# SuperScientificSoftwareLaboratory/DASP

Measured on AMD Instinct MI355X. Metric: SpMV GFLOP/s (f64), higher is better.
Workload: dtype f64; 1 GPU; HV15R synthetic stand-in (seeded; SuiteSparse dims/row statistics), A=1, x=1; rows=2017169, cols=2017169, nnz=275454726, partition=single GPU, generator_rev=26e32ff958e7, y_candidates=1

## Files before the change

dasp_amd/_lib.py:

```python
import ctypes as C
import os
import subprocess

_HERE = os.path.dirname(os.path.abspath(__file__))
SO_PATH = os.environ.get("DASP_AMD_SO") or os.path.join(_HERE, "libdasp_amd.so")


class DaspError(RuntimeError):
    def __init__(self, status, msg):
        super().__init__("dasp status %d: %s" % (status, msg))
        self.status = status


class Options(C.Structure):
    _fields_ = [
        ("threshold", C.c_double), ("block_longest", C.c_int), ("y_order", C.c_int), ("long_piece", C.c_int),
        ("host_threads", C.c_int), ("n_parts", C.c_int), ("part_bounds", C.POINTER(C.c_int)), ("part_stride", C.c_int),
        ("x_window", C.c_int), ("row_window", C.c_int), ("cid16", C.c_int), ("stream_policy", C.c_int),
        ("col_panels", C.c_int), ("slab_max_len", C.c_int), ("x_window_hybrid", C.c_int), ("piece_min_len", C.c_int),
        ("chunk_pairs", C.c_int), ("cid8", C.c_int), ("short_seg", C.c_int), ("row_tile_max", C.c_int), ("sort_columns", C.c_int),
        ("two_phase", C.c_int), ("tp_col_block", C.c_int), ("tp_row_block", C.c_int), ("long_cb", C.c_int),
        ("value_map", C.c_int),
    ]

    def _tp_exact_cell(self):
        return C.c_int.from_address(C.addressof(self) + Options.value_map.offset + C.sizeof(C.c_int))

    @property
    def tp_exact(self):
        return self._tp_exact_cell().value

    @tp_exact.setter
    def tp_exact(self, v):
        self._tp_exact_cell().value = int(v)


assert Options.value_map.offset + 2 * C.sizeof(C.c_int) <= C.sizeof(Options), "dasp_options_t::tp_exact must lie inside the Python mirror of the struct"


class Stats(C.Structure):
    _fields_ = [(n, C.c_int) for n in (
        "precision rowA colA nnzA short_row_1 common_13 short_row_3 short_row_4 short_row_2 row_long row_block "
        "row_zero nnz_short nnz_long origin_nnz_reg nnz_irreg rowloop").split()] + [
        ("fill0_nnz_short", C.c_longlong), ("fill0_nnz_long", C.c_longlong), ("fill0_nnz_reg", C.c_longlong),
        ("rate_fill0", C.c_double), ("data_X", C.c_longlong), ("data_origin1", C.c_longlong),
        ("n_med_blocks", C.c_int), ("n_long_pieces", C.c_int), ("n_long_multi", C.c_int), ("n_short_tiles", C.c_int),
        ("n_workgroups", C.c_int), ("pre_ms", C.c_double),
        ("x_window_on", C.c_int), ("n_windows", C.c_int), ("n_windows_lds", C.c_int), ("lds_bytes", C.c_int),
        ("row_window", C.c_int), ("window_nnz_frac", C.c_double), ("cid16_on", C.c_int),
        ("n_col_panels", C.c_int), ("x_window_hybrid", C.c_int), ("med_rows_as_pieces", C.c_int), ("chunk_pairs", C.c_int), ("cid8_chunks", C.c_int), ("short_seg", C.c_int),
        ("row_tile_max", C.c_int), ("n_row_tiles", C.c_int), ("row_tile_nnz", C.c_longlong),
        ("two_phase", C.c_int), ("tp_col_block", C.c_int), ("tp_row_blocks", C.c_int), ("tp_units", C.c_int), ("tp_segments", C.c_longlong), ("tp_seg_elems", C.c_int),
        ("lcb_rows", C.c_int), ("lcb_col_block", C.c_int), ("lcb_units", C.c_int), ("lcb_elems", C.c_longlong),
        ("ref_fill0_nnz_short", C.c_longlong), ("ref_fill0_nnz_long", C.c_longlong), ("ref_fill0_nnz_reg", C.c_longlong), ("ref_data_X", C.c_longlong),
        ("ref_nnz_irreg", C.c_int), ("ref_origin_nnz_reg", C.c_int), ("ref_blocknum", C.c_int), ("ref_warp_number", C.c_int), ("ref_rate_fill0", C.c_double)]

    def as_dict(self):
        return {n: getattr(self, n) for n, _ in self._fields_}


class MgInfo(C.Structure):
    _fields_ = [(n, C.c_int) for n in "precision n_gpus rank rowA colA row_begin row_end stride".split()] + [
        ("nnz_own", C.c_longlong), ("nnz_other", C.c_longlong), ("overlap", C.c_int), ("has_comm", C.c_int), ("square", C.c_int), ("stream_memops", C.c_int), ("fused_step", C.c_int), ("exchange", C.c_int)]

    def as_dict(self):
        return {n: getattr(self, n) for n, _ in self._fields_}


def build(force=False):
    src = os.path.join(_HERE, "csrc")
    if force:
        subprocess.check_call(["make", "-C", src, "-s", "clean"])
    subprocess.check_call(["make", "-C", src, "-s", "-j8", "all"])
    return SO_PATH


_lib = None


def _preload_hip_runtime():
    import importlib.util
    import sys
    if "torch" in sys.modules:
        return
    try:
        spec = importlib.util.find_spec("torch")
    except (ImportError, ValueError):
        spec = None
    if spec is None or not spec.origin:
        return
# ... 5 lines not shown
            pass


def lib():
    global _lib
    if _lib is not None:
        return _lib
    if not os.path.exists(SO_PATH):
        raise ImportError(
            "dasp_amd: %s is missing. Build it with `python -c 'import __graft_entry__ as g; g.build()'` "
            "(hipcc --offload-arch=gfx950). There is no fallback implementation." % SO_PATH)
    _preload_hip_runtime()
    L = C.CDLL(SO_PATH)
    ip, vp = C.POINTER(C.c_int), C.c_void_p
    L.dasp_last_error.restype = C.c_char_p
    L.dasp_version.restype = C.c_char_p
    L.dasp_free.argtypes = [vp]
    L.dasp_options_default.argtypes = [C.POINTER(Options)]
    L.dasp_mmio_allinone_f64.argtypes = [ip, ip, ip, ip, C.POINTER(ip), C.POINTER(ip), C.POINTER(C.POINTER(C.c_double)), C.c_char_p]
    L.dasp_mmio_allinone_f16.argtypes = [ip, ip, ip, ip, C.POINTER(ip), C.POINTER(ip), C.POINTER(C.POINTER(C.c_uint16)), C.c_char_p]
    L.dasp_csr_save.argtypes = [C.c_char_p, C.c_int, C.c_int, C.c_int, C.c_int, C.c_int, vp, vp, vp]
    L.dasp_csr_load.argtypes = [C.c_char_p, C.c_int, ip, ip, ip, ip, C.POINTER(ip), C.POINTER(ip), C.POINTER(vp)]
    L.dasp_plan_create.argtypes = [C.POINTER(vp), C.c_int, C.c_int, C.c_int, C.c_int, vp, vp, vp, C.POINTER(Options)]
    L.dasp_plan_create_device.argtypes = [C.POINTER(vp), C.c_int, C.c_int, C.c_int, C.c_int, vp, vp, vp, C.POINTER(Options)]
    L.dasp_plan_download_array.argtypes = [vp, C.c_char_p, vp, C.c_size_t]
    L.dasp_plan_destroy.argtypes = [vp]
    L.dasp_plan_save.argtypes = [vp, C.c_char_p]
    L.dasp_plan_load.argtypes = [C.POINTER(vp), C.c_char_p]
    L.dasp_plan_order.argtypes = [vp]
    L.dasp_plan_order.restype = ip
    L.dasp_plan_stats.argtypes = [vp, C.POINTER(Stats)]
    L.dasp_plan_y_order.argtypes = [vp]
    L.dasp_plan_x_len.argtypes = [vp]
    L.dasp_plan_x_len.restype = C.c_longlong
    L.dasp_plan_host_array.argtypes = [vp, C.c_char_p, C.POINTER(vp), ip]
    L.dasp_plan_host_array.restype = C.c_longlong
    L.dasp_plan_panel_count.argtypes = [vp]
    L.dasp_plan_panel.argtypes = [vp, C.c_int]
    L.dasp_plan_panel.restype = vp
    L.dasp_plan_panel_range.argtypes = [vp, C.c_int, ip, ip]
    L.dasp_plan_upload.argtypes = [vp]
    L.dasp_plan_drop_host.argtypes = [vp]
    L.dasp_plan_update_values.argtypes = [vp, vp, vp]
    L.dasp_plan_update_values_host.argtypes = [vp, vp]
    L.dasp_plan_value_map_slots.argtypes = [vp]
    L.dasp_plan_value_map_slots.restype = C.c_longlong
    if hasattr(L, "dasp_plan_csr_fetch_bytes"):
        L.dasp_plan_csr_fetch_bytes.argtypes = [vp]
        L.dasp_plan_csr_fetch_bytes.restype = C.c_longlong
    if hasattr(L, "dasp_plan_shared_ids"):
        L.dasp_plan_shared_ids.argtypes = [vp, C.POINTER(C.c_longlong), C.POINTER(C.c_longlong), ip]
        L.dasp_plan_shared_ids_export.argtypes = [vp, C.c_char_p, vp, C.c_size_t]
        L.dasp_plan_shared_ids_export.restype = C.c_longlong
    L.dasp_plan_set_stream_policy.argtypes = [vp, C.c_int]
    if hasattr(L, "dasp_plan_set_tp_exact"):
        L.dasp_plan_set_tp_exact.argtypes = [vp, C.c_int]
        L.dasp_plan_tp_exact.argtypes = [vp]
        L.dasp_tp_exact_dot_f16.argtypes = [vp, vp, C.c_longlong, C.c_int, C.c_uint16, C.POINTER(C.c_uint16)]
    if hasattr(L, "dasp_plan_set_hub_exact"):
        L.dasp_plan_set_hub_exact.argtypes = [vp, C.c_int]
        L.dasp_plan_hub_exact.argtypes = [vp]
    if hasattr(L, "dasp_plan_set_f32_vectors"):
        fp = C.POINTER(C.c_float)
        L.dasp_plan_set_f32_vectors.argtypes = [vp, C.c_int]
        L.dasp_plan_f32_vectors.argtypes = [vp]
        L.dasp_plan_spmv_f32.argtypes = [vp, fp, fp, vp]
        L.dasp_plan_spmv_acc_f32.argtypes = [vp, fp, fp, vp]
    if hasattr(L, "dasp_debug_plan_kernel"):
        L.dasp_debug_spmv_variant.argtypes = [C.c_int, C.c_uint]
        L.dasp_debug_spmv_variant.restype = C.c_char_p
        L.dasp_debug_plan_kernel.argtypes = [vp]
        L.dasp_debug_plan_kernel.restype = C.c_char_p
    L.dasp_plan_spmv.argtypes = [vp, vp, vp, vp]
    L.dasp_plan_spmv_acc.argtypes = [vp, vp, vp, vp]
    L.dasp_plan_time.argtypes = [vp, vp, vp, vp, C.c_int, C.c_int, C.POINTER(C.c_double), C.POINTER(C.c_double)]
    L.dasp_plan_time_each.argtypes = [vp, vp, vp, vp, C.c_int, C.c_int, vp]
    L.dasp_plan_time_graph.argtypes = [vp, vp, vp, vp, C.c_int, C.c_int, C.c_int, C.POINTER(C.c_double), C.POINTER(C.c_double)]
    L.dasp_spmv_all_f64.argtypes = [C.c_char_p, vp, vp, vp, vp, vp, vp, C.c_int, C.c_int, C.c_int, C.c_int, C.c_double, C.c_int]
    L.dasp_spmv_all_f16.argtypes = L.dasp_spmv_all_f64.argtypes
    L.dasp_partition_rows.argtypes = [C.c_int, vp, C.c_int, vp]
    L.dasp_selftest_mfma.argtypes = []
    L.dasp_plan_tune_placement.argtypes = [vp, C.c_int, vp, vp, C.POINTER(C.c_double), C.POINTER(C.c_double)]
    L.dasp_mg_unique_id.argtypes = [vp]
    L.dasp_mg_plan_create.argtypes = [C.POINTER(vp), C.c_int, C.c_int, C.c_int, C.c_int, C.c_int, vp, vp, vp, vp, C.POINTER(Options), C.c_int]
    L.dasp_mg_destroy.argtypes = [vp]
    L.dasp_mg_upload.argtypes = [vp]
    L.dasp_mg_comm_init.argtypes = [vp, vp]
    L.dasp_mg_set_x.argtypes = [vp, vp]
    L.dasp_mg_spmv.argtypes = [vp, vp]
    L.dasp_mg_product.argtypes = [vp, vp]
    L.dasp_mg_allgather.argtypes = [vp, vp]
    L.dasp_mg_wait.argtypes = [vp, vp]
    L.dasp_mg_get_y.argtypes = [vp, vp]
    L.dasp_mg_get_y_local.argtypes = [vp, vp]
    for f in (L.dasp_mg_y_local, L.dasp_mg_gathered, L.dasp_mg_x):
        f.argtypes = [vp]
        f.restype = vp
    L.dasp_mg_subplan.argtypes = [vp, C.c_int]
    L.dasp_mg_subplan.restype = vp
    L.dasp_mg_info.argtypes = [vp, C.POINTER(MgInfo)]
    L.dasp_mg_check.argtypes = [vp]
    L.dasp_mg_set_fused.argtypes = [vp, C.c_int]
    L.dasp_mg_set_fake_exchange.argtypes = [vp, C.c_int, C.c_int, vp]
    L.dasp_mg_push_export.argtypes = [vp, vp]
    L.dasp_mg_push_connect.argtypes = [vp, vp]
    L.dasp_mg_set_exchange.argtypes = [vp, C.c_int]
    L.dasp_mg_push_loopback.argtypes = [vp]
    L.dasp_mg_reserved_stream.argtypes = [vp, C.c_int]
    L.dasp_mg_reserved_stream.restype = vp
    L.dasp_synth_dims.argtypes = [C.c_char_p, C.c_double, ip, ip]
    L.dasp_synth_generator.argtypes = [C.c_char_p]
    L.dasp_synth_generator.restype = C.c_char_p
    L.dasp_synth_row_lengths.argtypes = [C.c_char_p, C.c_double, C.c_int, C.c_int, vp]
    L.dasp_synth_rows.argtypes = [C.c_char_p, C.c_double, C.c_int, C.c_int, vp, vp]
    _lib = L
    return L


def check(rc):
    if rc != 0:
        raise DaspError(rc, lib().dasp_last_error().decode("utf-8", "replace"))


EXPORTS = (
    "dasp_last_error dasp_version dasp_mmio_allinone_f64 dasp_mmio_allinone_f16 dasp_free dasp_csr_save dasp_csr_load dasp_options_default "
    "dasp_plan_create dasp_plan_create_device dasp_plan_download_array dasp_plan_destroy dasp_plan_save dasp_plan_load dasp_plan_order dasp_plan_stats dasp_plan_y_order dasp_plan_x_len dasp_plan_panel_count dasp_plan_panel dasp_plan_panel_range dasp_plan_host_array dasp_plan_upload dasp_plan_tune_placement "
    "dasp_plan_drop_host dasp_plan_update_values dasp_plan_update_values_host dasp_plan_value_map_slots dasp_plan_csr_fetch_bytes dasp_plan_shared_ids dasp_plan_shared_ids_export dasp_plan_set_stream_policy dasp_plan_set_tp_exact dasp_plan_tp_exact dasp_plan_set_hub_exact dasp_plan_hub_exact dasp_tp_exact_dot_f16 dasp_plan_spmv dasp_plan_spmv_acc dasp_plan_set_f32_vectors dasp_plan_f32_vectors dasp_plan_spmv_f32 dasp_plan_spmv_acc_f32 dasp_plan_time dasp_plan_time_each dasp_plan_time_graph dasp_spmv_all_f64 dasp_spmv_all_f16 dasp_partition_rows "
    "dasp_selftest_mfma dasp_synth_dims dasp_synth_generator dasp_synth_row_lengths dasp_synth_rows "
    "dasp_mg_unique_id dasp_mg_plan_create dasp_mg_destroy dasp_mg_upload dasp_mg_comm_init dasp_mg_set_x dasp_mg_spmv dasp_mg_product dasp_mg_allgather "
    "dasp_mg_wait dasp_mg_get_y dasp_mg_get_y_local dasp_mg_y_local dasp_mg_gathered dasp_mg_x dasp_mg_subplan dasp_mg_info dasp_mg_check dasp_mg_set_fused dasp_mg_set_fake_exchange "
    "dasp_mg_push_export dasp_mg_push_connect dasp_mg_set_exchange dasp_mg_push_loopback dasp_mg_reserved_stream").split()
```

dasp_amd/api.py:

```python
import ctypes as C
import os

import numpy as np

from . import _lib
from ._lib import DaspError, Options, Stats

Y_PERMUTED, Y_NATURAL = 0, 1


def _vp(a):
    return a.ctypes.data_as(C.c_void_p)


def _dtype(precision):
    if precision == 64:
        return np.float64
    if precision == 16:
        return np.float16
    raise ValueError("precision must be 64 or 16")


def mmio_allinone(filename, precision=64):
    L = _lib.lib()
    ip = C.POINTER(C.c_int)
    m, n, nnz, sym = C.c_int(), C.c_int(), C.c_int(), C.c_int()
    rp, ci = ip(), ip()
    if precision == 64:
        v = C.POINTER(C.c_double)()
        rc = L.dasp_mmio_allinone_f64(C.byref(m), C.byref(n), C.byref(nnz), C.byref(sym), C.byref(rp), C.byref(ci), C.byref(v), os.fsencode(filename))
    else:
        v = C.POINTER(C.c_uint16)()
        rc = L.dasp_mmio_allinone_f16(C.byref(m), C.byref(n), C.byref(nnz), C.byref(sym), C.byref(rp), C.byref(ci), C.byref(v), os.fsencode(filename))
    _lib.check(rc)
    k = nnz.value
    row_ptr = np.ctypeslib.as_array(rp, (m.value + 1,)).copy()
    col_idx = np.ctypeslib.as_array(ci, (max(k, 1),))[:k].copy()
    raw = np.ctypeslib.as_array(v, (max(k, 1),))[:k].copy()
    val = raw if precision == 64 else raw.view(np.float16)
    for q in (rp, ci, v):
        L.dasp_free(C.cast(q, C.c_void_p))
    return m.value, n.value, k, sym.value, row_ptr, col_idx, val


def csr_save(path, row_ptr, col_idx, val, n_cols, is_symmetric=0, precision=64):
    rp = np.ascontiguousarray(row_ptr, np.int32)
    ci = np.ascontiguousarray(col_idx, np.int32)
    v = np.ascontiguousarray(val, _dtype(precision))
    _lib.check(_lib.lib().dasp_csr_save(os.fsencode(path), precision, rp.size - 1, int(n_cols), int(ci.size), int(is_symmetric), _vp(rp), _vp(ci), _vp(v)))


def csr_load(path, precision=64):
    L = _lib.lib()
    ip = C.POINTER(C.c_int)
    m, n, nnz, sym = C.c_int(), C.c_int(), C.c_int(), C.c_int()
    rp, ci, v = ip(), ip(), C.c_void_p()
    _lib.check(L.dasp_csr_load(os.fsencode(path), precision, C.byref(m), C.byref(n), C.byref(nnz), C.byref(sym), C.byref(rp), C.byref(ci), C.byref(v)))
    k = nnz.value
    row_ptr = np.ctypeslib.as_array(rp, (m.value + 1,)).copy()
    col_idx = np.ctypeslib.as_array(ci, (max(k, 1),))[:k].copy()
    ct = C.c_double if precision == 64 else C.c_uint16
    raw = np.ctypeslib.as_array(C.cast(v, C.POINTER(ct)), (max(k, 1),))[:k].copy()
    val = raw if precision == 64 else raw.view(np.float16)
    for q in (C.cast(rp, C.c_void_p), C.cast(ci, C.c_void_p), v):
        L.dasp_free(q)
    return m.value, n.value, k, sym.value, row_ptr, col_idx, val


class Plan:

    def __init__(self, csrRowPtr, csrColIdx, csrVal, colA, precision=64, threshold=0.75, block_longest=256,
                 y_order=Y_PERMUTED, long_piece=0, host_threads=0, part_bounds=None, part_stride=0, x_window=0, row_window=0, cid16=0, stream_policy=0,
                 col_panels=0, slab_max_len=0, x_window_hybrid=0, piece_min_len=0, chunk_pairs=0, cid8=0, short_seg=0, row_tile_max=0, sort_columns=0,
                 two_phase=0, tp_col_block=0, tp_row_block=0, long_cb=0, value_map=0, tp_exact=0):
        L = _lib.lib()
        self.precision = precision
        dt = _dtype(precision)
        rp = np.ascontiguousarray(csrRowPtr, np.int32)
        ci = np.ascontiguousarray(csrColIdx, np.int32)
        v = np.ascontiguousarray(csrVal, dt)
        self.rowA, self.colA, self.nnzA = rp.size - 1, int(colA), int(ci.size)
        opt = Options()
        L.dasp_options_default(C.byref(opt))
        opt.threshold, opt.block_longest, opt.y_order = threshold, block_longest, y_order
        opt.long_piece, opt.host_threads = long_piece, host_threads
        opt.x_window, opt.row_window, opt.cid16, opt.stream_policy = x_window, row_window, cid16, stream_policy
        opt.col_panels, opt.slab_max_len, opt.x_window_hybrid, opt.piece_min_len = col_panels, slab_max_len, x_window_hybrid, piece_min_len
        opt.chunk_pairs, opt.cid8, opt.short_seg, opt.row_tile_max, opt.sort_columns = chunk_pairs, cid8, short_seg, row_tile_max, sort_columns
        opt.two_phase, opt.tp_col_block, opt.tp_row_block, opt.long_cb = two_phase, tp_col_block, tp_row_block, long_cb
        opt.value_map, opt.tp_exact = value_map, tp_exact
        self._pb = None
        if part_bounds is not None:
            self._pb = np.ascontiguousarray(part_bounds, np.int32)
            opt.n_parts = self._pb.size - 1
            opt.part_bounds = self._pb.ctypes.data_as(C.POINTER(C.c_int))
            opt.part_stride = int(part_stride)
        self._h = C.c_void_p()
        _lib.check(L.dasp_plan_create(C.byref(self._h), precision, self.rowA, self.colA, self.nnzA, _vp(rp), _vp(ci), _vp(v), C.byref(opt)))
        self.y_order = y_order
        self.x_len = self.colA if part_bounds is None else (self._pb.size - 1) * int(part_stride)

    @classmethod
    def from_device(cls, d_row_ptr, d_col_idx, d_val, rowA, colA, nnzA, precision=64, threshold=0.75, block_longest=256,
                    y_order=Y_PERMUTED, long_piece=0, part_bounds=None, part_stride=0, x_window=0, row_window=0, cid16=0, col_panels=0, slab_max_len=0,
                    x_window_hybrid=0, piece_min_len=0, chunk_pairs=0, cid8=0, short_seg=0, row_tile_max=0, sort_columns=0, two_phase=0, tp_col_block=0, tp_row_block=0, long_cb=0,
                    value_map=0, tp_exact=0):
        L = _lib.lib()
        self = cls.__new__(cls)
        self.precision, self.rowA, self.colA, self.nnzA = precision, int(rowA), int(colA), int(nnzA)
        opt = Options()
        L.dasp_options_default(C.byref(opt))
        opt.threshold, opt.block_longest, opt.y_order, opt.long_piece = threshold, block_longest, y_order, long_piece
        opt.x_window, opt.row_window, opt.cid16, opt.col_panels = x_window, row_window, cid16, col_panels
        opt.slab_max_len, opt.x_window_hybrid, opt.piece_min_len = slab_max_len, x_window_hybrid, piece_min_len
        opt.chunk_pairs, opt.cid8, opt.short_seg, opt.row_tile_max, opt.sort_columns = chunk_pairs, cid8, short_seg, row_tile_max, sort_columns
        opt.two_phase, opt.tp_col_block, opt.tp_row_block, opt.long_cb = two_phase, tp_col_block, tp_row_block, long_cb
        opt.value_map, opt.tp_exact = value_map, tp_exact
        self._pb = None
        if part_bounds is not None:
            self._pb = np.ascontiguousarray(part_bounds, np.int32)
            opt.n_parts, opt.part_stride = self._pb.size - 1, int(part_stride)
            opt.part_bounds = self._pb.ctypes.data_as(C.POINTER(C.c_int))
        self._h = C.c_void_p()
        _lib.check(L.dasp_plan_create_device(C.byref(self._h), precision, self.rowA, self.colA, self.nnzA, C.c_void_p(d_row_ptr),
                                             C.c_void_p(d_col_idx), C.c_void_p(d_val), C.byref(opt)))
        self.y_order = y_order
        self.x_len = int(L.dasp_plan_x_len(self._h))
        return self

    def device_array(self, name, count, dtype):
        out = np.empty(count, dtype)
        _lib.check(_lib.lib().dasp_plan_download_array(self._h, name.encode(), _vp(out), out.nbytes))
        return out

    def save(self, path):
        _lib.check(_lib.lib().dasp_plan_save(self._h, os.fsencode(path)))

    @classmethod
    def load(cls, path):
        self = cls.__new__(cls)
        self._h = C.c_void_p()
        self._pb = None
        _lib.check(_lib.lib().dasp_plan_load(C.byref(self._h), os.fsencode(path)))
        st = self.stats
        self.precision, self.rowA, self.colA, self.nnzA = st["precision"], st["rowA"], st["colA"], st["nnzA"]
        self.y_order = _lib.lib().dasp_plan_y_order(self._h)
        self.x_len = int(_lib.lib().dasp_plan_x_len(self._h))
        return self

    @property
    def order_rid(self):
        if self.rowA == 0:
            return np.zeros(0, np.int32)
        p = _lib.lib().dasp_plan_order(self._h)
        return np.ctypeslib.as_array(p, (max(self.rowA, 1),))[: self.rowA].copy()

    @property
    def stats(self):
        s = Stats()
        _lib.check(_lib.lib().dasp_plan_stats(self._h, C.byref(s)))
        return s.as_dict()

    @property
    def n_panels(self):
        return int(_lib.lib().dasp_plan_panel_count(self._h))

    def panel(self, k):
        L = _lib.lib()
        h = L.dasp_plan_panel(self._h, k)
        if not h:
# ... 14 lines not shown
            _lib.check(int(n))
        if name in ("med_cid16", "long_cid16", "rt_start", "tp_lrow", "tp_lcol", "lcb_lcol"):
            dt = np.uint16
        elif name.endswith("_val_map"):
            dt = np.uint32
        elif name == "rt_mask":
            dt = np.uint64
        elif name == "med_cid8":
            dt = np.uint8
        elif eb.value == 4:
            dt = np.int32
        else:
            dt = np.float64 if eb.value == 8 else np.float16
        if n == 0:
            return np.zeros(0, dt)
        buf = (C.c_char * (n * eb.value)).from_address(ptr.value)
        return np.frombuffer(buf, dtype=dt).copy()

    def upload(self):
        _lib.check(_lib.lib().dasp_plan_upload(self._h))
        return self

    def tune_placement(self, trials=0, dX=0, dY=0):
        a, b = C.c_double(), C.c_double()
        _lib.check(_lib.lib().dasp_plan_tune_placement(self._h, int(trials), C.c_void_p(dX or None), C.c_void_p(dY or None), C.byref(a), C.byref(b)))
        return a.value, b.value

    def drop_host(self):
        _lib.check(_lib.lib().dasp_plan_drop_host(self._h))

    def update_values(self, csrVal):
        v = np.ascontiguousarray(csrVal, _dtype(self.precision))
        if v.size != self.nnzA:
            raise ValueError("update_values: %d values for a plan of %d nonzeros" % (v.size, self.nnzA))
        _lib.check(_lib.lib().dasp_plan_update_values_host(self._h, _vp(v)))

    def update_values_device(self, d_val, stream=0):
        _lib.check(_lib.lib().dasp_plan_update_values(self._h, C.c_void_p(d_val), C.c_void_p(stream)))

    @property
    def csr_fetch_bytes(self):
        n = int(_lib.lib().dasp_plan_csr_fetch_bytes(self._h))
        if n < 0:
            _lib.check(n)
        return n

    def shared_ids(self):
        pb, sb, use = C.c_longlong(0), C.c_longlong(0), C.c_int(0)
        rc = _lib.lib().dasp_plan_shared_ids(self._h, C.byref(pb), C.byref(sb), C.byref(use))
        if rc < 0:
            _lib.check(rc)
        return {"available": bool(rc), "paired_id_bytes": int(pb.value), "shared_bytes": int(sb.value), "in_use": bool(use.value)}

    def shared_ids_export(self):
        out = []
        for what in (b"plane", b"table"):
            n = int(_lib.lib().dasp_plan_shared_ids_export(self._h, what, None, 0))
            if n < 0:
                _lib.check(n)
            a = np.empty(n // 4, np.uint32)
            n2 = int(_lib.lib().dasp_plan_shared_ids_export(self._h, what, a.ctypes.data_as(C.c_void_p), a.nbytes))
            if n2 < 0:
                _lib.check(n2)
            out.append(a)
        return out[0], out[1].reshape(-1, 4)

    @property
    def value_map_slots(self):
        n = int(_lib.lib().dasp_plan_value_map_slots(self._h))
        if n < 0:
            _lib.check(n)
        return n

    def kernel_variant(self):
        name = _lib.lib().dasp_debug_plan_kernel(self._h)
        if name is None:
            raise _lib.DaspError(-22, _lib.lib().dasp_last_error().decode("utf-8", "replace"))
        return name.decode()

    def set_stream_policy(self, policy):
        _lib.check(_lib.lib().dasp_plan_set_stream_policy(self._h, int(policy)))

    def set_tp_exact(self, on):
        _lib.check(_lib.lib().dasp_plan_set_tp_exact(self._h, int(on)))

    @property
    def tp_exact(self):
        return int(_lib.lib().dasp_plan_tp_exact(self._h))

    def set_hub_exact(self, on):
        _lib.check(_lib.lib().dasp_plan_set_hub_exact(self._h, int(on)))

    @property
    def hub_exact(self):
        return int(_lib.lib().dasp_plan_hub_exact(self._h))

    def spmv(self, dX, dY, stream=0, accumulate=False):
        f = _lib.lib().dasp_plan_spmv_acc if accumulate else _lib.lib().dasp_plan_spmv
        _lib.check(f(self._h, C.c_void_p(dX), C.c_void_p(dY), C.c_void_p(stream)))

    def set_f32_vectors(self, on):
        _lib.check(_lib.lib().dasp_plan_set_f32_vectors(self._h, int(on)))

    @property
    def f32_vectors(self):
        return int(_lib.lib().dasp_plan_f32_vectors(self._h))
# ... 110 lines not shown
```

dasp_amd/csrc/capi.cpp:

```cpp
#include <hip/hip_runtime_api.h>

#include <algorithm>
#include <cstdio>
#include <cstdlib>
#include <cstring>
#include <exception>
#include <memory>
#include <new>
#include <string>
#include <sys/stat.h>
#include <vector>

#include "plan.hpp"
#include "device.hpp"
#include "tp_exact.hpp"

namespace dasp {
const char *last_error_cstr();
int upload_plan(Plan &p);
int tune_placement(Plan &p, int trials, const void *dX, void *dY, double *ms_first, double *ms_kept);
int launch_spmv(Plan &p, const void *dX, void *dY, void *stream, bool accumulate);
int time_spmv_each(Plan &p, const void *dX, void *dY, void *stream, int warmup, int iters, float *ms_each);
int time_spmv(Plan &p, const void *dX, void *dY, void *stream, int warmup, int iters, double *wall_ms, double *event_ms);
int time_spmv_graph(Plan &p, const void *dX, void *dY, void *stream, int warmup, int iters, int batch, double *wall_ms, double *event_ms);
// ... 25 lines not shown
    std::memset(o, 0, sizeof *o);
    o->threshold = 0.75;
    o->block_longest = 256;
    o->y_order = DASP_Y_PERMUTED;
}

int dasp_mmio_allinone_f64(int *m, int *n, int *nnz, int *isSymmetric, int **csrRowPtr, int **csrColIdx,
                           double **csrVal, const char *filename)
{
    void *v = nullptr;
    int rc = guarded("dasp_mmio_allinone_f64", [&] { return load_mtx(filename, 64, m, n, nnz, isSymmetric, csrRowPtr, csrColIdx, &v); });
    if (rc == DASP_OK) *csrVal = static_cast<double *>(v);
    return rc;
}

int dasp_mmio_allinone_f16(int *m, int *n, int *nnz, int *isSymmetric, int **csrRowPtr, int **csrColIdx,
                           uint16_t **csrVal, const char *filename)
{
    void *v = nullptr;
    int rc = guarded("dasp_mmio_allinone_f16", [&] { return load_mtx(filename, 16, m, n, nnz, isSymmetric, csrRowPtr, csrColIdx, &v); });
    if (rc == DASP_OK) *csrVal = static_cast<uint16_t *>(v);
    return rc;
}

int dasp_csr_save(const char *path, int precision, int m, int n, int nnz, int isSymmetric, const int *csrRowPtr,
                  const int *csrColIdx, const void *csrVal)
{
    return guarded("dasp_csr_save", [&] { return save_csr_bin(path, precision, m, n, nnz, isSymmetric, csrRowPtr, csrColIdx, csrVal); });
}

int dasp_csr_load(const char *path, int precision, int *m, int *n, int *nnz, int *isSymmetric, int **csrRowPtr,
                  int **csrColIdx, void **csrVal)
{
    return guarded("dasp_csr_load", [&] { return load_csr_bin(path, precision, m, n, nnz, isSymmetric, csrRowPtr, csrColIdx, csrVal); });
}

static int normalise_options(Plan &p, const dasp_options_t *opt, int colA)
{
    if (opt) p.opt = *opt; else dasp_options_default(&p.opt);
    if (!(p.opt.threshold > 0)) p.opt.threshold = 0.75;
    if (p.opt.block_longest < 6) p.opt.block_longest = 256;
    if (p.opt.n_parts > 0) {
        if (!p.opt.part_bounds || p.opt.part_stride <= 0) { set_error("bad column partition"); return DASP_ERR_ARG; }
        p.part_bounds.assign(p.opt.part_bounds, p.opt.part_bounds + p.opt.n_parts + 1);
        if (p.part_bounds.front() != 0 || p.part_bounds.back() != colA) { set_error("part_bounds must span [0,colA]"); return DASP_ERR_ARG; }
        for (int g = 0; g < p.opt.n_parts; ++g)
            if (p.part_bounds[g + 1] < p.part_bounds[g] || p.part_bounds[g + 1] - p.part_bounds[g] > p.opt.part_stride) {
                set_error("part_bounds not monotone or wider than part_stride"); return DASP_ERR_ARG;
            }
        p.opt.part_bounds = p.part_bounds.data();
    } else { p.opt.n_parts = 0; p.opt.part_bounds = nullptr; }
    if (p.opt.value_map != 0 && p.opt.value_map != 1) { set_error("value_map must be 0 or 1"); return DASP_ERR_ARG; }
    if (p.opt.tp_exact != 0 && p.opt.tp_exact != 1) { set_error("tp_exact must be 0 or 1"); return DASP_ERR_ARG; }
    return DASP_OK;
}

int dasp_plan_create(dasp_plan_t **out, int precision, int rowA, int colA, int nnzA, const int *rp, const int *ci,
                     const void *val, const dasp_options_t *opt)
{
    if (!out) return DASP_ERR_ARG;
    *out = nullptr;
    if ((precision != 64 && precision != 16) || rowA < 0 || colA < 0 || nnzA < 0 || !rp || (nnzA > 0 && (!ci || !val))) {
        set_error("dasp_plan_create: bad arguments");
        return DASP_ERR_ARG;
    }
    return guarded("dasp_plan_create", [&] {
        std::unique_ptr<dasp_plan> h(new dasp_plan());
        Plan &p = h->impl;
        p.precision = precision; p.m = rowA; p.n = colA; p.nnz = nnzA;
        if (int rc = normalise_options(p, opt, colA)) return rc;
        if (int rc = build_plan(p, rp, ci, val)) return rc;
        if (int rc = set_tp_exact(p, p.opt.tp_exact)) return rc;
        *out = h.release();
        return (int)DASP_OK;
    });
}

int dasp_plan_create_device(dasp_plan_t **out, int precision, int rowA, int colA, int nnzA, const int *dRowPtr, const int *dColIdx,
                            const void *dVal, const dasp_options_t *opt)
{
    if (!out) return DASP_ERR_ARG;
    *out = nullptr;
    if ((precision != 64 && precision != 16) || rowA < 0 || colA < 0 || nnzA < 0 || !dRowPtr || (nnzA > 0 && (!dColIdx || !dVal))) {
        set_error("dasp_plan_create_device: bad arguments");
        return DASP_ERR_ARG;
    }
    return guarded("dasp_plan_create_device", [&] {
        std::vector<int> rp((size_t)rowA + 1);
        if (hipMemcpy(rp.data(), dRowPtr, sizeof(int) * ((size_t)rowA + 1), hipMemcpyDeviceToHost) != hipSuccess) {
            set_error("cannot read the device row pointer (no HIP device, or not a device pointer)");
            return (int)DASP_ERR_HIP;
        }
        std::unique_ptr<dasp_plan> h(new dasp_plan());
        Plan &p = h->impl;
        p.precision = precision; p.m = rowA; p.n = colA; p.nnz = nnzA;
        if (int rc = normalise_options(p, opt, colA)) return rc;
        const DevCsr dev{dRowPtr, dColIdx, dVal};
        if (int rc = build_plan(p, rp.data(), nullptr, nullptr, &dev)) return rc;
        if (int rc = set_tp_exact(p, p.opt.tp_exact)) return rc;
        *out = h.release();
        return (int)DASP_OK;
    });
}

int dasp_plan_download_array(dasp_plan_t *plan, const char *name, void *dst, size_t bytes)
{
// ... 121 lines not shown
    if (n == "rt_ptr") return ints(p.rt_ptr);
    if (n == "rt_start") { *ptr = p.rt_start.data(); *elem_bytes = 2; return (long long)p.rt_start.size(); }
    if (n == "rt_mask") { *ptr = p.rt_mask.data(); *elem_bytes = 8; return (long long)p.rt_mask.size(); }
    if (n == "lcb_row_dst") return ints(p.lcb.row_dst);
    if (n == "lcb_row_id") return ints(p.lcb.row_id);
    if (n == "lcb_ptr") return ints(p.lcb.ptr);
    if (n == "lcb_unit") return ints(p.lcb.unit);
    if (n == "lcb_val") return vals(p.lcb.val);
    if (n == "lcb_lcol") { *ptr = p.lcb.lcol.data(); *elem_bytes = 2; return (long long)p.lcb.lcol.size(); }
    if (n == "tp_rb_row0") return ints(p.tp.rb_row0);
    if (n == "tp_rb_seg0") return ints(p.tp.rb_seg0);
    if (n == "tp_unit") return ints(p.tp.unit);
    if (n == "tp_dst") return ints(p.tp.dst);
    if (n == "tp_val") return vals(p.tp.val);
    if (n == "tp_lrow") { *ptr = p.tp.lrow.data(); *elem_bytes = 2; return (long long)p.tp.lrow.size(); }
    if (n == "tp_lcol") { *ptr = p.tp.lcol.data(); *elem_bytes = 2; return (long long)p.tp.lcol.size(); }
    if (n == "short_groups") {
        static thread_local std::vector<int> flat;
        flat.clear();
        for (int g = 0; g < kNumShortGroups; ++g) {
            const ShortGroup &G = p.grp[g];
            const int row[15] = {G.len, G.count, G.tiles, G.tile0, (int)(G.elem_off & 0xffffffffll), (int)(G.elem_off >> 32),
                                 G.map.split, G.map.base[0], G.map.base[1], G.map.grp[0], G.map.grp[1], G.map.off[0], G.map.off[1], G.seg, G.rpt};
            flat.insert(flat.end(), row, row + 15);
        }
        return ints(flat);
    }
    set_error("unknown host array: " + n);
    return DASP_ERR_ARG;
}

long long dasp_plan_csr_fetch_bytes(const dasp_plan_t *plan) { return plan ? plan->impl.csr_fetch_bytes : (long long)DASP_ERR_ARG; }

int dasp_plan_shared_ids(const dasp_plan_t *plan, long long *paired_id_bytes, long long *shared_bytes, int *in_use)
{
    if (!plan) return DASP_ERR_ARG;
    const Plan &p = plan->impl;
    if (paired_id_bytes) *paired_id_bytes = 0;
    if (shared_bytes) *shared_bytes = 0;
    if (in_use) *in_use = p.dev && p.sh_in_use ? 1 : 0;
    return guarded("dasp_plan_shared_ids", [&] {
        long long pb = 0, sb = 0;
        if (!p.sh_known) {
            SharedIds sh;
            (void)derive_shared_ids(p, sh);
            p.sh_paired_bytes = sh.paired_id_bytes; p.sh_shared_bytes = sh.shared_bytes; p.sh_known = true;
        }
        pb = p.sh_paired_bytes; sb = p.sh_shared_bytes;
        if (pb == 0) return 0;
        if (paired_id_bytes) *paired_id_bytes = pb;
        if (shared_bytes) *shared_bytes = sb;
        return 1;
    });
}

long long dasp_plan_shared_ids_export(const dasp_plan_t *plan, const char *what, void *dst, size_t bytes)
{
    if (!plan || !what) return DASP_ERR_ARG;
    long long need = 0;
    const int rc = guarded("dasp_plan_shared_ids_export", [&] {
        const bool plane = std::strcmp(what, "plane") == 0;
        if (!plane && std::strcmp(what, "table") != 0) { set_error("dasp_plan_shared_ids_export: \"plane\" or \"table\""); return (int)DASP_ERR_ARG; }
        SharedIds sh;
        if (!derive_shared_ids(plan->impl, sh)) { set_error("the plan has no shared id plane (f64 with 16-bit ids, host arrays present, at least one pipelined block)"); return (int)DASP_ERR_STATE; }
        const std::vector<uint32_t> &v = plane ? sh.plane : sh.table;
        need = (long long)v.size() * 4;
        if (dst && bytes >= (size_t)need && need > 0) std::memcpy(dst, v.data(), (size_t)need);
        return (int)DASP_OK;
    });
    return rc != DASP_OK ? (long long)rc : need;
}

int dasp_plan_upload(dasp_plan_t *plan)
{
    if (!plan) return DASP_ERR_ARG;
    return guarded("dasp_plan_upload", [&] { return upload_plan(plan->impl); });
}

int dasp_plan_tune_placement(dasp_plan_t *plan, int trials, const void *dX, void *dY, double *ms_first, double *ms_kept)
{
    if (!plan) return DASP_ERR_ARG;
    if (!plan->impl.dev) { set_error("plan not uploaded"); return DASP_ERR_STATE; }
    return guarded("dasp_plan_tune_placement", [&] { return tune_placement(plan->impl, trials, dX, dY, ms_first, ms_kept); });
}

int dasp_plan_drop_host(dasp_plan_t *plan)
{
    if (!plan) return DASP_ERR_ARG;
    Plan &p = plan->impl;
    if (!p.dev) { set_error("upload the plan before dropping its host arrays"); return DASP_ERR_STATE; }
    auto dropc = [](raw_vector<char> &v) { raw_vector<char>().swap(v); };
    auto dropi = [](raw_vector<int> &v) { raw_vector<int>().swap(v); };
    dropc(p.long_val); dropi(p.long_cid); raw_vector<uint16_t>().swap(p.long_cid16); dropc(p.med_val); dropi(p.med_cid); raw_vector<uint16_t>().swap(p.med_cid16); raw_vector<uint8_t>().swap(p.med_cid8);
    dropc(p.irr_val); dropi(p.irr_cid); dropc(p.short_val); dropi(p.short_cid); dropc(p.rt_val); dropi(p.rt_cid);
    dropc(p.lcb.val); raw_vector<uint16_t>().swap(p.lcb.lcol);
    dropc(p.tp.val); raw_vector<uint16_t>().swap(p.tp.lrow); raw_vector<uint16_t>().swap(p.tp.lcol); std::vector<int>().swap(p.tp.dst);
    for (auto *m : {&p.long_map, &p.med_map, &p.irr_map, &p.short_map, &p.rt_map, &p.tp.map, &p.lcb.map}) std::vector<uint32_t>().swap(*m);
    p.host_dropped = true;
    for (auto &h : p.panels) if (int rc = dasp_plan_drop_host(h.get())) return rc;
    return DASP_OK;
}

int dasp_plan_set_stream_policy(dasp_plan_t *plan, int policy)
{
    if (!plan) return DASP_ERR_ARG;
    return set_stream_policy(plan->impl, policy);
// ... 212 lines not shown
```

dasp_amd/csrc/devpack.hip:

```cpp
#include <hip/hip_runtime.h>
#include <hipcub/hipcub.hpp>

#include <memory>
#include <thread>

#include <algorithm>
#include <chrono>
#include <cstdio>
#include <cstdlib>
#include <cstring>
#include <string>
#include <type_traits>
#include <vector>

#include "device.hpp"

namespace dasp {

#define HIP_TRYP(expr)                                                                         \
    do {                                                                                       \
        hipError_t e_ = (expr);                                                                \
        if (e_ != hipSuccess) {                                                                \
            set_error(std::string(#expr) + ": " + hipGetErrorString(e_));                      \
            return e_ == hipErrorNoDevice ? DASP_ERR_NO_DEVICE : DASP_ERR_HIP;                 \
// ... 89 lines not shown
__global__ void k_iota1(unsigned *out, long long n)
{
    for (long long i = (long long)blockIdx.x * blockDim.x + threadIdx.x; i < n; i += (long long)gridDim.x * blockDim.x) out[i] = (unsigned)(i + 1);
}

template <class T>
__global__ void k_pack_long(const int *rp, const int *ci, const T *val, const int *ridL, const long long *startL, int nlong, RemapDev remap,
                            T *lv, int *lc, const unsigned *src, unsigned *lm )
{
    const int lane = threadIdx.x & 63, i = blockIdx.x * (blockDim.x >> 6) + (threadIdx.x >> 6);
    if (i >= nlong) return;
    const int r = ridL[i], a0 = rp[r], len = rp[r + 1] - a0;
    const long long at = startL[i], padded = startL[i + 1] - at;
    for (long long j = lane; j < padded; j += 64) {
        const bool in = j < len;
        lv[at + j] = in ? val[a0 + j] : (T)0;
        lc[at + j] = in ? remap(ci[a0 + j]) : -1;
        if (lm) lm[at + j] = in ? map_of(src, a0 + j) : 0u;
    }
}

__global__ void k_long_cid16(const int *lc, const int *piece_ptr, int *piece_c16, int np, int CH, int *lbase, unsigned short *lc16)
{
    const int lane = threadIdx.x & 63, q = blockIdx.x * (blockDim.x >> 6) + (threadIdx.x >> 6);
    if (q >= np) return;
    const int e0 = piece_ptr[q], e1 = piece_ptr[q + 1], c0 = piece_c16[2 * q];
    bool narrow = true;
    for (int e = e0, c = c0; e < e1; e += CH, ++c) {
        int lo = 2147483647, hi = -1;
        for (int j = e + lane; j < min(e + CH, e1); j += 64) { const int col = lc[j]; if (col >= 0) { lo = min(lo, col); hi = max(hi, col); } }
        for (int d = 32; d > 0; d >>= 1) { lo = min(lo, __shfl_xor(lo, d)); hi = max(hi, __shfl_xor(hi, d)); }
        const int b = hi < 0 ? 0 : lo;
        if (lane == 0) lbase[c] = b;
        if (hi >= 0 && (long long)hi - lo > 65534) narrow = false;
        for (int j = e + lane; j < min(e + CH, e1); j += 64) { const int col = lc[j]; lc16[j] = col < 0 ? kLongPad16 : (unsigned short)(col - b); }
    }
    narrow = narrow && e1 - e0 >= kLong16MinChunks * CH;
    if (lane == 0) piece_c16[2 * q + 1] = narrow ? 1 : 0;
    if (!narrow) for (int j = e0 + lane; j < e1; j += 64) lc16[j] = 0;
}

template <class T, bool C16>
__global__ void k_pack_medium(const int *rp, const int *ci, const T *val, const int *ridM, const int *lenM, const int *med_ptr,
                              const int *irr_ptr, int nmed, int nb, RemapDev remap, T *mv, int *mc, unsigned short *mc16, int *mbase,
                              T *iv, int *ic, int pair_mode, const int *c8ptr, unsigned char *mc8, int *korig,
                              const int *win_cmin, const int *win_len, int bpw ,
                              const unsigned *src, unsigned *mm, unsigned *im )
{
    constexpr int K = sizeof(T) == 8 ? 4 : 16, CH = kMedRows * K, VPL = CH / 64;
    const int lane = threadIdx.x & 63, b = blockIdx.x * (blockDim.x >> 6) + (threadIdx.x >> 6);
    if (b >= nb) return;
    const int c0 = med_ptr[b], nc = med_ptr[b + 1] - c0;
    const int r0 = b * kMedRows;
    const int nt_b = (irr_ptr[r0 + 1] - irr_ptr[r0] + K - 1) / K;
    const int npair = med_npair(nc, nt_b, (int)sizeof(T), pair_mode);
    const bool oneshot = med_oneshot64(nc, nt_b);
    const int rr = lane & 15, kq = lane >> 4, r = r0 + rr;
    const bool row_ok = r < nmed;
    const int a0 = row_ok ? rp[ridM[r]] : 0, len = row_ok ? lenM[r] : 0;
    int n8 = 0, a8 = 0, a16 = 0; size_t e8 = 0, e16 = (size_t)c0 * CH;
    if constexpr (C16) { n8 = c8ptr[b + 1] - c8ptr[b]; e8 = (size_t)c8ptr[b] * CH; e16 = ((size_t)c0 - (size_t)c8ptr[b]) * CH; }
    for (int c = 0; c < nc; ++c) {
        int col[VPL]; T v[VPL]; unsigned ms[VPL];
        int lo = 2147483647, hi = -1;
#pragma unroll
        for (int q = 0; q < VPL; ++q) {
            const int i = c * K + (VPL == 1 ? kq : 4 * kq + q);
            const bool in = row_ok && i < len;
            v[q] = in ? val[a0 + i] : (T)0;
            col[q] = in ? remap(ci[a0 + i]) : -1;
            ms[q] = in && mm ? map_of(src, a0 + i) : 0u;
            if (in) { lo = min(lo, col[q]); hi = max(hi, col[q]); }
        }
        if constexpr (C16) {
            lo = wave_min(lo); hi = wave_max(hi);
            const bool narrow = c < npair && c < 64 && a8 < n8 && hi >= 0 && hi - lo <= 254;
            if (lo == 2147483647) lo = 0;
            if (bpw > 0 && win_len[b / bpw] > 0) lo = win_cmin[b / bpw];
            const int pos = c >= npair ? c : narrow ? a8++ : n8 + a16++;
            if (lane == 0) { mbase[c0 + pos] = lo; korig[c0 + pos] = c; }
            const size_t at = (size_t)c0 * CH + med_elem_index(npair, pos, lane, 0, VPL, CH);
#pragma unroll
            for (int q = 0; q < VPL; ++q) {
                mv[at + q] = v[q];
                if (mm) mm[at + q] = ms[q];
                if (pos < n8) mc8[e8 + med_cid8_index(pos, lane, CH, oneshot)] = col[q] < 0 ? (unsigned char)0xFF : (unsigned char)(col[q] - lo);
                else mc16[e16 + med_elem_index(npair - n8, pos - n8, lane, q, VPL, CH)] = col[q] < 0 ? (unsigned short)0xFFFF : (unsigned short)(col[q] - lo);
            }
        } else {
            const size_t at = (size_t)c0 * CH + med_elem_index(npair, c, lane, 0, VPL, CH);
#pragma unroll
            for (int q = 0; q < VPL; ++q) { mv[at + q] = v[q]; mc[at + q] = col[q]; if (mm) mm[at + q] = ms[q]; }
        }
    }
    if (row_ok) {
        const int t0 = irr_ptr[r], tl = irr_ptr[r + 1] - t0;
        for (int j = kq; j < tl; j += 4) {
            iv[t0 + j] = val[a0 + len - tl + j]; ic[t0 + j] = remap(ci[a0 + len - tl + j]);
            if (im) im[t0 + j] = map_of(src, a0 + len - tl + j);
        }
    }
}

template <class T>
__global__ void k_pack_short(const int *rp, const int *ci, const T *val, const int *list, int count, int tiles, int L, long long elem_off,
                             int SR, int seg, RemapDev remap, T *sv, int *sc, const unsigned *src, unsigned *sm )
{
    const long long n = (long long)tiles * short_tile_elems(seg != 0, L, SR);
    for (long long e = (long long)blockIdx.x * blockDim.x + threadIdx.x; e < n; e += (long long)gridDim.x * blockDim.x) {
        long long t; int k; bool in;
        if (seg) {
// ... 1262 lines not shown
```

dasp_amd/csrc/multigpu.cpp:

```cpp
#include <hip/hip_runtime_api.h>
#include <hip/hip_ext.h>
#include <rccl/rccl.h>

#include <dlfcn.h>

#include <algorithm>
#include <chrono>
#include <cstdlib>
#include <cstring>
#include <exception>
#include <memory>
#include <mutex>
#include <new>
#include <string>
#include <thread>
#include <vector>

#include <unistd.h>

#include "plan.hpp"
#include "device.hpp"
#include "mgx.hpp"

using namespace dasp;
// ... 215 lines not shown
        if (xg && xg != yg) (void)hipFree(xg);
        if (own) dasp_plan_destroy(own);
        if (other) dasp_plan_destroy(other);
    }
};

namespace {

template <class T>
void split_by_owner(int m, const int *rp, const int *ci, const T *val, int lo, int hi, int threads,
                    std::vector<int> &rpO, std::vector<int> &ciO, std::vector<T> &vO,
                    std::vector<int> &rpR, std::vector<int> &ciR, std::vector<T> &vR)
{
    rpO.assign((size_t)m + 1, 0); rpR.assign((size_t)m + 1, 0);
    auto par = [&](auto f) {
        const int parts = std::max(1, std::min(threads, m / 4096 + 1));
        std::vector<std::thread> th;
        for (int t = 0; t < parts; ++t) {
            const int b = (int)((long long)m * t / parts), e = (int)((long long)m * (t + 1) / parts);
            th.emplace_back([=] { f(b, e); });
        }
        for (auto &x : th) x.join();
    };
    par([&](int b, int e) {
        for (int i = b; i < e; ++i) {
            int o = 0;
            for (int j = rp[i]; j < rp[i + 1]; ++j) o += ci[j] >= lo && ci[j] < hi;
            rpO[(size_t)i + 1] = o; rpR[(size_t)i + 1] = rp[i + 1] - rp[i] - o;
        }
    });
    for (int i = 0; i < m; ++i) { rpO[(size_t)i + 1] += rpO[i]; rpR[(size_t)i + 1] += rpR[i]; }
    ciO.resize((size_t)rpO[m]); vO.resize((size_t)rpO[m]); ciR.resize((size_t)rpR[m]); vR.resize((size_t)rpR[m]);
    par([&](int b, int e) {
        for (int i = b; i < e; ++i) {
            int o = rpO[i], r = rpR[i];
            for (int j = rp[i]; j < rp[i + 1]; ++j) {
                if (ci[j] >= lo && ci[j] < hi) { ciO[(size_t)o] = ci[j] - lo; vO[(size_t)o++] = val[j]; }
                else { ciR[(size_t)r] = ci[j]; vR[(size_t)r++] = val[j]; }
            }
        }
    });
}

template <class T>
int create_impl(dasp_mg_plan &g, const int *rp, const int *ci, const T *val, const dasp_options_t *user)
{
    const int m = g.rows();
    const int lo = g.bounds[(size_t)g.rank], hi = g.bounds[(size_t)g.rank + 1];
    dasp_options_t opt;
    if (user) opt = *user; else dasp_options_default(&opt);
    opt.y_order = DASP_Y_NATURAL;
    opt.short_seg = -1;
    opt.two_phase = -1;
    opt.n_parts = 0; opt.part_bounds = nullptr; opt.part_stride = 0;
    opt.tp_exact = 0;
    opt.value_map = 0;
    const int nnz = rp[m];
    if (!g.square) {
        g.nnz_own = nnz; g.nnz_other = 0;
        return dasp_plan_create(&g.own, g.precision, m, g.colA, nnz, rp, ci, val, &opt);
    }
    dasp_options_t part = opt;
    part.n_parts = g.world; part.part_bounds = g.bounds.data(); part.part_stride = g.stride;
    if (!g.overlap) {
        g.nnz_own = nnz; g.nnz_other = 0;
        return dasp_plan_create(&g.own, g.precision, m, g.colA, nnz, rp, ci, val, &part);
    }
    if (g.step2) {
        std::vector<unsigned char> has((size_t)std::max(m, 1), 0);
        long long other = 0;
        for (int i = 0; i < m; ++i) {
            int o = 0;
            for (int j = rp[i]; j < rp[i + 1]; ++j) o += !(ci[j] >= lo && ci[j] < hi);
            has[(size_t)i] = o > 0; other += o;
        }
        g.nnz_own = nnz - other; g.nnz_other = other;
        if (int rc = dasp_plan_create(&g.own, g.precision, m, g.colA, nnz, rp, ci, val, &part)) return rc;
        const Plan &P = g.own->impl;
        if (g.precision == 64 && P.panels.empty() && !P.windowed && P.opt.y_order == DASP_Y_NATURAL) {
            double hot_at = 1.0;
            if (const char *e = std::getenv("DASP_MG_HOT_AT")) hot_at = std::max(0.0, std::min(1.0, std::atof(e)));
            mg_step_marks(P, has.data(), g.mark, g.blk_order, hot_at);
            const int n_pieces = (int)P.piece_dst.size(), wg_long = (n_pieces + kWavesPerWG - 1) / kWavesPerWG;
            const int wg_med = (P.stats.n_med_blocks + kWavesPerWG - 1) / kWavesPerWG;
            int first_hot_med = wg_long + wg_med;
            for (int w = wg_long; w < wg_long + wg_med; ++w) if (g.mark[(size_t)w]) { first_hot_med = w; break; }
            g.wg_list.clear(); g.wg_list.reserve(g.mark.size());
            for (int w = 0; w < first_hot_med; ++w) if (!g.mark[(size_t)w]) g.wg_list.push_back(w);
            g.n_free2 = (int)g.wg_list.size();
            for (size_t w = 0; w < g.mark.size(); ++w) if (g.mark[w]) g.wg_list.push_back((int)w);
            g.n_marked2 = (int)g.wg_list.size() - g.n_free2;
            for (int w = first_hot_med; w < (int)g.mark.size(); ++w) if (!g.mark[(size_t)w]) g.wg_list.push_back(w);
        }
        return DASP_OK;
    }
    std::vector<int> rpO, ciO, rpR, ciR;
    std::vector<T> vO, vR;
    split_by_owner<T>(m, rp, ci, val, lo, hi, resolve_threads(opt.host_threads), rpO, ciO, vO, rpR, ciR, vR);
    g.nnz_own = rpO[(size_t)m]; g.nnz_other = rpR[(size_t)m];
    static const int zero = 0;
    if (int rc = dasp_plan_create(&g.own, g.precision, m, g.stride, rpO[(size_t)m], rpO.data(), ciO.empty() ? &zero : ciO.data(),
                                  vO.empty() ? static_cast<const void *>(&zero) : vO.data(), &opt)) return rc;
    if (part.cid16 == 0 && g.precision == 64 && g.own->impl.cid16) part.cid16 = 1;
    if (g.nnz_other > 0)
        if (int rc = dasp_plan_create(&g.other, g.precision, m, g.colA, rpR[(size_t)m], rpR.data(), ciR.data(), vR.data(), &part)) return rc;
    if (g.other && g.precision == 64 && g.own->impl.panels.empty() && !g.own->impl.windowed && g.own->impl.opt.y_order == DASP_Y_NATURAL) {
// ... 773 lines not shown
```

dasp_amd/csrc/plan.cpp:

```cpp
#include "plan.hpp"

#include <algorithm>
#include <array>
#include <atomic>
#include <chrono>
#include <cstdio>
#include <cstdlib>
#include <cstring>
#include <condition_variable>
#include <functional>
#include <mutex>
#include <thread>

namespace dasp {

static thread_local std::string g_err;
void set_error(const std::string &s) { g_err = s; }
const char *last_error_cstr() { return g_err.c_str(); }

int resolve_threads(int requested)
{
    if (requested > 0) return requested;
    unsigned hc = std::thread::hardware_concurrency();
    if (hc == 0) hc = 1;
// ... 326 lines not shown
    g.fill0_reg = reg; g.nnz_irreg = (int)irr;
    const long long stored = g.fill0_short + g.fill0_long + g.nnz_irreg + g.fill0_reg;
    g.rate_fill0 = nnz > 0 ? (double)(stored - nnz) / nnz : 0.0;
    const long long sv = f16 ? 2 : 8;
    g.data_X = (long long)(m + n) * sv + g.fill0_long * (sv + 4) + (long long)g.warp_number * sv + (long long)(lenL.size() + 1) * 4 + g.fill0_short * (sv + 4) +
               g.fill0_reg * (sv + 4) + (long long)(g.blocknum + 1) * 4 + (long long)(f16 ? (g.nnz_irreg + 1) / 2 * 2 : g.nnz_irreg) * (sv + 4) +
               (long long)(row_block + 1) * 4;
    return g;
}

namespace {
struct LapTimer {
    using clk = std::chrono::steady_clock;
    const char *fmt;
    const clk::time_point t_begin = clk::now();
    const bool verbose = std::getenv("DASP_VERBOSE") != nullptr;
    clk::time_point tick = t_begin;
    explicit LapTimer(const char *f) : fmt(f) {}
    void operator()(const char *what) { if (verbose) { auto now = clk::now(); std::fprintf(stderr, fmt, what, std::chrono::duration<double>(now - tick).count()); tick = now; } }
    double ms() const { return std::chrono::duration<double, std::milli>(clk::now() - t_begin).count(); }
};

template <class T> struct Build {
    Plan &p;
    const int *rp, *ci;
    const T *val;
    const DevCsr *dev;
    const Geometry geo;
    const int m, nnz, threads;
    const bool f16;
    const bool meta_only;
    const bool pack;
    const bool natural, mapped;
    Remap remap;
    LapTimer lap{"[dasp plan] %-28s %.3f s\n"};

    std::vector<int> rid1, rid2, rid3, rid4, rid0;
    int n1 = 0, n3 = 0;
    int n2 = 0, n4 = 0, nz0 = 0, n1_all = 0, n3_all = 0, c13 = 0;
    int row_long = 0;
    int row_block = 0;
    int nnz_short = 0;
    long long nnz_long = 0;
    std::vector<int> ridL;
    raw_vector<int> ridM_in;
    raw_vector<int> ridM, lenM;
    RefGeometry refg;
    int mfma_rows = 0;
    std::vector<std::vector<int>> slab_rows;
    const std::vector<int> *glist[kNumShortGroups] = {};
    double window_frac = 0.0;
    int nsp = 0;
    int rows_as_pieces = 0;
    std::vector<long long> startL;
    int nb = 0;
    long long n_reg = 0;
    int nnz_irreg = 0;

    Build(Plan &p_, const int *rp_, const int *ci_, const T *val_, const DevCsr *dev_, bool meta_only_)
        : p(p_), rp(rp_), ci(ci_), val(val_), dev(dev_), geo(p_.geo), m(p_.m), nnz(p_.nnz), threads(resolve_threads(p_.opt.host_threads)), f16(p_.precision == 16),
          meta_only(meta_only_), pack(!dev_ && !meta_only_), natural(p_.opt.y_order == DASP_Y_NATURAL), mapped(natural && !p_.dst_map.empty())
    {
        remap.n_parts = p.opt.n_parts; remap.stride = p.opt.part_stride; remap.b = p.part_bounds.data();
    }
    Build(const Build &) = delete;
    Build &operator=(const Build &) = delete;
    CsrProbe probe() const { return CsrProbe{p, rp, ci, dev, remap, threads}; }
    int rowdst(int row) const { return mapped ? p.dst_map[row] : row; }
    int ydst(int slot) const { return natural ? rowdst(p.order[slot]) : slot; }
};

bool row_ptr_ends_ok(const int *rp, int m, int nnz)
{
    if (rp[0] != 0 || rp[m] != nnz) { set_error("csrRowPtr[0] != 0 or csrRowPtr[rowA] != nnzA"); return false; }
    return true;
}
}

template <class T> static int validate_csr(Build<T> &bld)
{
    Plan &p = bld.p;
    const int *rp = bld.rp, *ci = bld.ci;
    const DevCsr *dev = bld.dev;
    const int m = bld.m, nnz = bld.nnz, threads = bld.threads;
    if (!row_ptr_ends_ok(rp, m, nnz)) return DASP_ERR_ARG;
    std::atomic<int> bad{0};
    parallel_for(m, threads, 1 << 16, [&](long long b, long long e) {
        for (long long i = b; i < e; ++i) if (rp[i + 1] < rp[i]) { bad = 1; return; }
    });
    const int ncol = p.n;
    if (dev) { if (!bad) { const int rc = devpack_validate(p, *dev); if (rc == DASP_ERR_ARG) bad = 2; else if (rc != DASP_OK) return rc; } }
    else parallel_for(nnz, threads, 1 << 18, [&](long long b, long long e) {
        for (long long i = b; i < e; ++i) if ((unsigned)ci[i] >= (unsigned)ncol) { bad = 2; return; }
    });
    if (bad) { set_error(bad == 1 ? "csrRowPtr not monotone" : "column index out of range"); return DASP_ERR_ARG; }
    bld.lap("validate");
    return DASP_OK;
}

template <class T> struct SortedCsr {
    raw_vector<int> ci;
    raw_vector<T> val;
    raw_vector<uint32_t> src;
    DevCsr dev{nullptr, nullptr, nullptr};
    std::vector<std::shared_ptr<void>> keep;
};
// ... 600 lines not shown
    }

    bld.lap("window decision");
    return DASP_OK;
}

template <class T> static int medium_rows_as_pieces(Build<T> &bld)
{
    Plan &p = bld.p;
    const Geometry &geo = bld.geo;
    const int *rp = bld.rp;
    const int nnz = bld.nnz;
    const bool f16 = bld.f16, meta_only = bld.meta_only;
    std::vector<int> &ridL = bld.ridL;
    raw_vector<int> &ridM = bld.ridM, &lenM = bld.lenM, &ridM_in = bld.ridM_in;
    int &mfma_rows = bld.mfma_rows, &nsp = bld.nsp;
    nsp = 0;
    if (mfma_rows > 0 && !meta_only && p.opt.piece_min_len >= 0 && !p.windowed) {
        int Tmin = p.opt.piece_min_len > 0 ? std::max(5, p.opt.piece_min_len) : 0;
        if (Tmin == 0) {
            const double est_us = (double)nnz * (geo.vbytes + 4) / 5.0e6;
            const int shot = f16 ? 2 : 8, batch = f16 ? 2 : 4;
            auto batches = [&](int L) { const int st = ceil_div(L, geo.med_k); return st <= shot ? 1 : ceil_div(st, batch); };
            const int allowed = std::max(2, (int)(0.25 * est_us / 0.8));
            if (batches(lenM[0]) > allowed) {
                int Lmax = lenM[0];
                while (Lmax > 5 && batches(Lmax) > allowed) --Lmax;
                Tmin = Lmax + 1;
            }
        }
        if (Tmin > 0) {
            const bool forced = p.opt.piece_min_len > 0;
            int cnt = 0; long long k = 0;
            while (cnt < mfma_rows && lenM[cnt] >= Tmin && (forced || (k + lenM[cnt]) * 100 <= 15ll * nnz)) { k += lenM[cnt]; ++cnt; }
            while (cnt > 0 && cnt < mfma_rows && lenM[cnt] == lenM[cnt - 1]) --cnt;
            nsp = cnt;
        }
    }
    if (nsp > 0) {
        const int Tcut = lenM[nsp - 1];
        ridL.insert(ridL.end(), ridM.begin(), ridM.begin() + nsp);
        ridM.erase(ridM.begin(), ridM.begin() + nsp); lenM.erase(lenM.begin(), lenM.begin() + nsp);
        raw_vector<int> keep; keep.reserve(ridM_in.size());
        for (int r : ridM_in) if (rp[r + 1] - rp[r] < Tcut) keep.push_back(r);
        ridM_in.swap(keep);
        mfma_rows -= nsp;
    }
    bld.rows_as_pieces = bld.row_long + nsp;
    p.med_slot0 = bld.rows_as_pieces;
    p.n_mfma_rows = mfma_rows;
    return DASP_OK;
}

template <class T> static int pack_long(Build<T> &bld)
{
    Plan &p = bld.p;
    const Geometry &geo = bld.geo;
    const int *rp = bld.rp, *ci = bld.ci;
    const T *val = bld.val;
    const Remap remap = bld.remap;
    const int nnz = bld.nnz, threads = bld.threads, rows_as_pieces = bld.rows_as_pieces;
    const bool f16 = bld.f16, pack = bld.pack;
    const std::vector<int> &ridL = bld.ridL;
    std::vector<long long> &startL = bld.startL;
    long long nnz_pieces = 0;
    for (int r : ridL) nnz_pieces += rp[r + 1] - rp[r];
    int piece = p.opt.long_piece > 0 ? p.opt.long_piece : 1024;
    if (p.opt.long_piece <= 0) {
        int longest = 0;
        for (int r : ridL) longest = std::max(longest, rp[r + 1] - rp[r]);
        const int one_piece = ab_knobs().one_piece_max;
        const double chain_us = 0.35 * (double)longest / (double)(geo.chunk * (f16 ? kMedBatch16 : kMedBatch64));
        const double rest_us = 4.0 + 3.0 + (double)nnz * (double)(geo.vbytes + 4) / 5.0e6;
        if ((nnz_pieces <= 2000000 && longest <= 16384 && chain_us <= rest_us) || longest <= one_piece) piece = std::max(piece, longest);
    }
    piece = std::max(geo.chunk, ceil_div(piece, geo.chunk) * geo.chunk);
    {
        std::vector<long long> start((size_t)rows_as_pieces + 1, 0);
        for (int i = 0; i < rows_as_pieces; ++i) {
            const int len = rp[ridL[i] + 1] - rp[ridL[i]];
            start[i + 1] = start[i] + (long long)ceil_div(len, kLongAlign) * kLongAlign;
        }
        const long long total = start[rows_as_pieces];
        if (total >= (1LL << 31)) { set_error("long-row segment exceeds 2^31 elements"); return DASP_ERR_ARG; }
        p.cnt_long = (size_t)total;
        startL = start;
        if (pack) {
        p.long_val.resize((size_t)total * sizeof(T));
        p.long_cid.resize((size_t)total);
        if (p.value_map) p.long_map.assign((size_t)total, 0u);
        }
        p.piece_ptr.clear(); p.piece_dst.clear(); p.multi_ptr.assign(1, 0); p.multi_dst.clear();
        int n_partial = 0;
        for (int i = 0; i < rows_as_pieces; ++i) {
            const long long lp = start[i + 1] - start[i];
            const int np = (int)((lp + piece - 1) / piece);
            for (int q = 0; q < np; ++q) {
                p.piece_ptr.push_back((int)(start[i] + (long long)q * piece));
                p.piece_dst.push_back(np == 1 ? bld.ydst(i) : ~(n_partial++));
            }
            if (np > 1) { p.multi_ptr.push_back(n_partial); p.multi_dst.push_back(bld.ydst(i)); }
        }
        p.piece_ptr.push_back((int)total);
        T *lv = reinterpret_cast<T *>(p.long_val.data());
        if (pack) parallel_for(total, threads, 1 << 16, [&](long long b, long long e) {
            long long i = std::upper_bound(start.begin(), start.end(), b) - start.begin() - 1;
            for (; i < rows_as_pieces && start[i] < e; ++i) {
                const int r = ridL[i], len = rp[r + 1] - rp[r];
                const long long s0 = std::max(b, start[i]), s1 = std::min(e, start[i + 1]);
                const long long real_end = std::min(s1, start[i] + len);
                const long long src = (long long)rp[r] - start[i];
                for (long long j = s0; j < real_end; ++j) { lv[j] = val[src + j]; p.long_cid[(size_t)j] = remap(ci[src + j]); }
                if (p.value_map) for (long long j = s0; j < real_end; ++j) p.long_map[(size_t)j] = map_entry(p, src + j);
                for (long long j = std::max(s0, real_end); j < s1; ++j) { lv[j] = (T)0; p.long_cid[(size_t)j] = -1; }
            }
        });
        {
            const int CHL = geo.chunk, np_all = (int)p.piece_dst.size();
            p.piece_c16.assign((size_t)2 * (size_t)np_all, 0);
            long long nchunk = 0;
            for (int q = 0; q < np_all; ++q) { p.piece_c16[(size_t)2 * q] = (int)nchunk; nchunk += ceil_div(p.piece_ptr[(size_t)q + 1] - p.piece_ptr[(size_t)q], CHL); }
            if (pack) {
                p.long_base.assign((size_t)nchunk, 0);
                p.long_cid16.resize((size_t)total);
                parallel_for(np_all, threads, 16, [&](long long q0, long long q1) {
                    for (long long q = q0; q < q1; ++q) {
                        const int e0 = p.piece_ptr[(size_t)q], e1 = p.piece_ptr[(size_t)q + 1], c0 = p.piece_c16[(size_t)2 * q];
                        bool narrow = true;
                        for (int e = e0, c = c0; e < e1; e += CHL, ++c) {
// ... 20 lines not shown
    return DASP_OK;
}

template <class T> static int split_medium_chunks(Build<T> &bld)
{
    Plan &p = bld.p;
    const Geometry &geo = bld.geo;
    const int nnz = bld.nnz, threads = bld.threads, mfma_rows = bld.mfma_rows;
    const bool f16 = bld.f16, meta_only = bld.meta_only, pack = bld.pack;
    const double threshold = p.opt.threshold;
    const raw_vector<int> &ridM = bld.ridM, &lenM = bld.lenM;
    const int K = geo.med_k, CH = geo.chunk;
    const int nb = bld.nb = ceil_div(mfma_rows, kMedRows);
    std::vector<int> nchunks((size_t)nb + 1, 0);
    p.irr_ptr.assign((size_t)mfma_rows + 1, 0);
    std::vector<int> nchunks16((size_t)nb + 1, 0);
    const bool try16 = p.opt.cid16 >= 0 && !meta_only;
    const bool try8 = try16 && !f16 && p.opt.cid8 >= 0;
    std::vector<unsigned long long> narrow_mask(try8 ? (size_t)nb : 0, 0ull);
    parallel_for(nb, threads, 256, [&](long long b0, long long b1) {
        for (long long b = b0; b < b1; ++b) {
            const int r0 = (int)b * kMedRows, r1 = std::min(mfma_rows, r0 + kMedRows);
            int k = 0;
            for (;; ++k) {
                int fill = 0;
                for (int r = r0; r < r1; ++r) fill += std::min(K, std::max(0, lenM[r] - K * k));
                if (!(fill >= threshold * CH) || fill == 0) break;
            }
            nchunks[b] = k; nchunks16[b] = k;
        }
    });
    if (try16) { if (int rc = bld.probe().chunk_spans(ridM, lenM, nchunks, K, nchunks16.data(), try8 ? narrow_mask.data() : nullptr)) return rc; }
    {
        long long e32 = 0, e16 = 0;
        for (int b = 0; b < nb; ++b) { e32 += nchunks[b]; e16 += nchunks16[b]; }
        const bool streams = (long long)nnz * (geo.vbytes + 4) > (p.windowed ? kStreamBytes : (16ll << 20));
        const bool rel1 = p.windowed && !p.win_hybrid && p.opt.x_window != -2 && p.lds_bytes / geo.vbytes <= 65534;
        p.cid16 = try16 && e32 > 0 && (p.opt.cid16 > 0 || ((streams || rel1) && (double)e16 >= 0.97 * (double)e32));
        if (p.cid16) nchunks.swap(nchunks16);
        p.win_rel16 = p.cid16 && p.windowed && !p.win_hybrid && p.lds_bytes / geo.vbytes <= 65534;
    }
    parallel_for(nb, threads, 1 << 12, [&](long long b0, long long b1) {
        for (long long b = b0; b < b1; ++b) {
            const int r0 = (int)b * kMedRows, r1 = std::min(mfma_rows, r0 + kMedRows);
            for (int r = r0; r < r1; ++r) p.irr_ptr[(size_t)r] = std::max(0, lenM[(size_t)r] - K * nchunks[(size_t)b]);
        }
    });
    p.pair_mode = p.windowed || p.opt.chunk_pairs < 0 ? 0 : p.opt.chunk_pairs > 0 ? std::min(2, p.opt.chunk_pairs)
                                                                     : ((long long)nnz * (geo.vbytes + 4) > 4 * kStreamBytes ? 2 : 1);
    std::vector<int> n8of((size_t)nb + 1, 0);
    if (try8 && p.cid16 && p.pair_mode > 0) {
        long long total8 = 0, total = 0;
        for (int b = 0; b < nb; ++b) {
            const int nt = (p.irr_ptr[(size_t)b * kMedRows] + K - 1) / K, npair = med_npair(nchunks[b], nt, geo.vbytes, p.pair_mode);
            const unsigned long long in = npair >= 64 ? ~0ull : ((1ull << npair) - 1);
            n8of[b] = p.opt.cid8 == 0 && med_oneshot64(nchunks[b], nt) ? 0 : med_n8(__builtin_popcountll(narrow_mask[(size_t)b] & in), nchunks[b], nt);
            total8 += n8of[b]; total += nchunks[b];
        }
        if (p.opt.cid8 == 0 && total8 * 10 < total) std::fill(n8of.begin(), n8of.end(), 0);
        if (p.opt.cid8 == 0 && p.opt.cid16 == 0 && (long long)nnz * (geo.vbytes + 4) <= (64ll << 20)) std::fill(n8of.begin(), n8of.end(), 0);
    }
    bld.lap("chunk split (+cid16 spans)");
    p.med_ptr.assign((size_t)nb + 1, 0);
    {
        long long run = 0;
        for (int b = 0; b < nb; ++b) { p.med_ptr[b] = (int)run; run += nchunks[b]; }
        if (run >= (1LL << 31) / 1) { set_error("too many medium chunks"); return DASP_ERR_ARG; }
        p.med_ptr[nb] = (int)run;
        const int sparts = (int)std::max<long long>(1, std::min<long long>(threads, ((long long)mfma_rows + (1 << 16) - 1) >> 16));
        std::vector<long long> psum((size_t)sparts + 1, 0);
        parallel_for(sparts, sparts, 1, [&](long long p0, long long p1) {
            for (long long q = p0; q < p1; ++q) {
                long long a = 0;
                for (long long r = (long long)mfma_rows * q / sparts, e = (long long)mfma_rows * (q + 1) / sparts; r < e; ++r) a += p.irr_ptr[(size_t)r];
                psum[(size_t)q + 1] = a;
            }
        });
        for (int q = 0; q < sparts; ++q) psum[(size_t)q + 1] += psum[(size_t)q];
        parallel_for(sparts, sparts, 1, [&](long long p0, long long p1) {
            for (long long q = p0; q < p1; ++q) {
                long long t = psum[(size_t)q];
                for (long long r = (long long)mfma_rows * q / sparts, e = (long long)mfma_rows * (q + 1) / sparts; r < e; ++r) { const int v = p.irr_ptr[(size_t)r]; p.irr_ptr[(size_t)r] = (int)t; t += v; }
            }
        });
        long long t = psum[(size_t)sparts];
        p.irr_ptr[mfma_rows] = (int)t;
    }
    bld.n_reg = (long long)p.med_ptr[nb] * CH;
    bld.nnz_irreg = p.irr_ptr[mfma_rows];
    p.cnt_reg = (size_t)bld.n_reg; p.cnt_irr = (size_t)bld.nnz_irreg;
    p.med_base.assign(p.cid16 && pack ? (size_t)p.med_ptr[nb] : 0, 0);
    p.med_c8ptr.clear(); p.med_korig.clear(); p.med_cid8.clear(); p.cnt_reg8 = 0;
    if (p.cid16) {
        p.med_c8ptr.assign((size_t)nb + 1, 0);
        for (int b = 0; b < nb; ++b) p.med_c8ptr[(size_t)b + 1] = p.med_c8ptr[b] + n8of[b];
        p.cnt_reg8 = (size_t)p.med_c8ptr[nb] * CH;
        p.med_korig.assign((size_t)p.med_ptr[nb], 0);
    }
    return DASP_OK;
}

template <class T> static int pack_medium(Build<T> &bld)
{
    if (!bld.pack) { bld.lap("pack medium"); return DASP_OK; }
    Plan &p = bld.p;
    const Geometry &geo = bld.geo;
    const int *rp = bld.rp, *ci = bld.ci;
    const T *val = bld.val;
    const Remap remap = bld.remap;
    const int threads = bld.threads, mfma_rows = bld.mfma_rows, nb = bld.nb, nnz_irreg = bld.nnz_irreg;
    const long long n_reg = bld.n_reg;
    const bool f16 = bld.f16;
    const raw_vector<int> &ridM = bld.ridM, &lenM = bld.lenM;
    const int K = geo.med_k, CH = geo.chunk, VPL = geo.chunk / 64;
    p.med_val.resize((size_t)n_reg * sizeof(T));
    p.med_cid.resize(p.cid16 ? 0 : (size_t)n_reg);
    p.med_cid16.resize(p.cid16 ? (size_t)n_reg - p.cnt_reg8 : 0);
    p.med_cid8.resize(p.cnt_reg8);
    p.irr_val.resize((size_t)nnz_irreg * sizeof(T));
    p.irr_cid.resize((size_t)nnz_irreg);
    if (p.value_map) { p.med_map.assign((size_t)n_reg, 0u); p.irr_map.assign((size_t)nnz_irreg, 0u); }
    T *mv = reinterpret_cast<T *>(p.med_val.data());
    T *iv = reinterpret_cast<T *>(p.irr_val.data());
    parallel_for(nb, threads, 64, [&](long long b0, long long b1) {
        std::vector<int> pos_of, lo_of;
        for (long long b = b0; b < b1; ++b) {
            const int nc = p.med_ptr[b + 1] - p.med_ptr[b];
            const size_t base = (size_t)p.med_ptr[b] * CH;
            const int r0 = (int)b * kMedRows, r1 = std::min(mfma_rows, r0 + kMedRows);
            const int nt_b = (p.irr_ptr[r0 + 1] - p.irr_ptr[r0] + K - 1) / K;
            const int npair = med_npair(nc, nt_b, geo.vbytes, p.pair_mode);
            const bool oneshot = med_oneshot64(nc, nt_b);
            const int n8 = p.cid16 ? p.med_c8ptr[b + 1] - p.med_c8ptr[b] : 0;
            const size_t e8 = p.cid16 ? (size_t)p.med_c8ptr[b] * CH : 0;
            const size_t e16 = p.cid16 ? ((size_t)p.med_ptr[b] - (size_t)p.med_c8ptr[b]) * CH : 0;
            pos_of.assign((size_t)nc + 1, 0); lo_of.assign((size_t)nc + 1, 0);
            if (p.cid16) {
                int a8 = 0, a16 = 0;
                for (int c = 0; c < nc; ++c) {
                    int lo = 2147483647, hi = -1;
                    for (int r = r0; r < r1; ++r) {
                        const int a0 = rp[ridM[r]], i0 = c * K, i1 = std::min(lenM[r], i0 + K);
                        for (int i = i0; i < i1; ++i) { const int col = remap(ci[a0 + i]); lo = std::min(lo, col); hi = std::max(hi, col); }
                    }
                    const bool narrow = c < npair && c < 64 && a8 < n8 && hi >= 0 && hi - lo <= 254;
                    lo_of[c] = lo == 2147483647 ? 0 : lo;
                    if (p.win_rel16) { const size_t w = (size_t)b / (size_t)(p.row_window / kMedRows); if (p.win_len[w] > 0) lo_of[c] = p.win_cmin[w]; }
                    pos_of[c] = c >= npair ? c : narrow ? a8++ : n8 + a16++;
                }
                for (int c = 0; c < nc; ++c) {
                    p.med_base[(size_t)p.med_ptr[b] + pos_of[c]] = lo_of[c];
                    p.med_korig[(size_t)p.med_ptr[b] + pos_of[c]] = c;
                }
            } else for (int c = 0; c < nc; ++c) pos_of[c] = c;
            {
                const size_t n = (size_t)nc * CH;
                std::fill(mv + base, mv + base + n, (T)0);
                if (p.cid16) {
                    std::fill(p.med_cid8.begin() + e8, p.med_cid8.begin() + e8 + (size_t)n8 * CH, (uint8_t)0xFF);
                    std::fill(p.med_cid16.begin() + e16, p.med_cid16.begin() + e16 + (size_t)(nc - n8) * CH, (uint16_t)0xFFFF);
                } else std::fill(p.med_cid.begin() + base, p.med_cid.begin() + base + n, -1);
            }
            for (int r = r0; r < r1; ++r) {
                const int rr = r - r0, row = ridM[r], len = lenM[r], a0 = rp[row];
                const int nreg = std::min(len, nc * K);
                for (int i = 0; i < nreg; ++i) {
                    const int c = i / K, kk = i % K, q = pos_of[c];
                    const int lane = f16 ? (kk / 4) * kMedRows + rr : kk * kMedRows + rr, j = f16 ? kk % 4 : 0;
                    const size_t at = base + med_elem_index(npair, q, lane, j, VPL, CH);
                    mv[at] = val[a0 + i];
                    if (p.value_map) p.med_map[at] = map_entry(p, a0 + i);
                    const int col = remap(ci[a0 + i]);
                    if (!p.cid16) p.med_cid[at] = col;
                    else if (q < n8) p.med_cid8[e8 + med_cid8_index(q, lane, CH, oneshot)] = (uint8_t)(col - lo_of[c]);
                    else p.med_cid16[e16 + med_elem_index(npair - n8, q - n8, lane, j, VPL, CH)] = (uint16_t)(col - lo_of[c]);
                }
                const int t0 = p.irr_ptr[r], tl = p.irr_ptr[r + 1] - t0;
                for (int j = 0; j < tl; ++j) {
                    iv[t0 + j] = val[a0 + len - tl + j];
                    if (p.value_map) p.irr_map[(size_t)(t0 + j)] = map_entry(p, a0 + len - tl + j);
                    p.irr_cid[t0 + j] = remap(ci[a0 + len - tl + j]);
                }
            }
// ... 44 lines not shown
    p.short_val.resize((size_t)off * sizeof(T));
    p.short_cid.resize((size_t)off);
    if (p.value_map) p.short_map.assign((size_t)off, 0u);
    T *sv = reinterpret_cast<T *>(p.short_val.data());
    for (int g = 0; g < kNumShortGroups; ++g) {
        const ShortGroup &G = p.grp[g];
        if (G.tiles == 0 || G.len == 0) continue;
        const size_t te = (size_t)short_tile_elems(G.seg != 0, G.len, SR);
        const size_t t0 = (size_t)G.elem_off + (G.seg && G.len == 3 ? 0 : (size_t)(G.tiles - 1) * te), t1 = (size_t)G.elem_off + (size_t)G.tiles * te;
        std::fill(sv + t0, sv + t1, (T)0);
        std::fill(p.short_cid.begin() + t0, p.short_cid.begin() + t1, -1);
    }
    for (int g = 0; g < kNumShortGroups; ++g) {
        const ShortGroup &G = p.grp[g];
        if (G.len == 0 || G.count == 0) continue;
        const std::vector<int> &list = *glist[g];
        parallel_for(G.count, threads, 1 << 14, [&](long long b, long long e) {
            for (long long t = b; t < e; ++t) {
                const int row = list[t], a0 = rp[row];
                for (int k = 0; k < G.len; ++k) {
                    const size_t at = (size_t)G.elem_off + short_elem_index(G.seg != 0, G.len, SR, t, k);
                    sv[at] = val[a0 + k];
                    if (p.value_map) p.short_map[at] = map_entry(p, a0 + k);
                    p.short_cid[at] = remap(ci[a0 + k]);
                }
            }
        });
    }
    }

    bld.lap("pack short");
    return DASP_OK;
}

template <class T> static int fill_stats(Build<T> &bld)
{
    Plan &p = bld.p;
    const Geometry &geo = bld.geo;
    const RefGeometry &refg = bld.refg;
    const int m = bld.m, nnz = bld.nnz, n1 = bld.n1, n2 = bld.n2, n3 = bld.n3, n4 = bld.n4, nz0 = bld.nz0, c13 = bld.c13, nsp = bld.nsp;
    const int row_long = bld.row_long, row_block = bld.row_block, mfma_rows = bld.mfma_rows, nb = bld.nb;
    const int nnz_short = bld.nnz_short, nnz_irreg = bld.nnz_irreg;
    const long long nnz_long = bld.nnz_long, n_reg = bld.n_reg;
    const bool natural = bld.natural;
    const double window_frac = bld.window_frac;
    dasp_stats_t &s = p.stats;
    std::memset(&s, 0, sizeof s);
    s.precision = p.precision; s.rowA = m; s.colA = p.n; s.nnzA = nnz;
    s.short_row_1 = n1; s.common_13 = c13; s.short_row_3 = n3; s.short_row_4 = n4; s.short_row_2 = n2;
    s.short_seg = 0;
    for (int g = 0; g < kNumShortGroups; ++g) s.short_seg |= p.grp[g].seg;
    s.row_long = row_long; s.row_block = row_block; s.row_zero = nz0; s.med_rows_as_pieces = nsp; s.chunk_pairs = p.pair_mode; s.cid8_chunks = p.med_c8ptr.empty() ? 0 : p.med_c8ptr.back();
    s.nnz_short = nnz_short; s.nnz_long = (int)nnz_long; s.nnz_irreg = nnz_irreg;
    s.origin_nnz_reg = nnz - nnz_irreg - (int)nnz_long - nnz_short;
    s.rowloop = mfma_rows < 59990 ? 1 : (mfma_rows < 400000 ? 2 : 4);
    s.fill0_nnz_short = (long long)p.cnt_short;
    s.fill0_nnz_long = (long long)p.cnt_long;
    s.fill0_nnz_reg = n_reg;
    const long long stored = s.fill0_nnz_short + s.fill0_nnz_long + s.fill0_nnz_reg + nnz_irreg;
    s.rate_fill0 = nnz > 0 ? (double)(stored - nnz) / nnz : 0.0;
    const long long sv = geo.vbytes;
    s.cid16_on = p.cid16 ? 1 : 0;
    s.data_X = (long long)(m + p.n) * sv + stored * (sv + 4) - (p.cid16 ? 2 * n_reg - 4ll * p.med_ptr[nb] : 0) - (long long)p.cnt_reg8 +
               (long long)(p.piece_ptr.size() + p.piece_dst.size() + p.multi_ptr.size() + p.multi_dst.size()) * 4 +
               (long long)(p.med_ptr.size() + p.irr_ptr.size()) * 4 + (natural ? (long long)m * 4 : 0) +
               (long long)(p.med_dst.size() + 2 * p.win_len.size()) * 4;
    s.data_origin1 = (long long)(nnz + p.n + m) * sv + (long long)nnz * 4 + (long long)(m + 1) * 4;
    s.ref_fill0_nnz_short = refg.fill0_short; s.ref_fill0_nnz_long = refg.fill0_long; s.ref_fill0_nnz_reg = refg.fill0_reg; s.ref_data_X = refg.data_X;
    s.ref_nnz_irreg = refg.nnz_irreg; s.ref_origin_nnz_reg = nnz - refg.nnz_irreg - (int)nnz_long - nnz_short; s.ref_blocknum = refg.blocknum;
    s.ref_warp_number = refg.warp_number; s.ref_rate_fill0 = refg.rate_fill0;
    s.n_med_blocks = nb;
    s.n_long_pieces = (int)p.piece_dst.size();
    s.n_long_multi = (int)p.multi_dst.size();
    s.n_short_tiles = 0;
    for (int g = 0; g < kNumShortGroups; ++g) s.n_short_tiles += p.grp[g].tiles;
    s.n_workgroups = ceil_div(s.n_long_pieces, kWavesPerWG) + ceil_div(nb, kWavesPerWG) + ceil_div(s.n_short_tiles, kWavesPerWG);
    s.x_window_on = p.windowed ? 1 : 0; s.n_windows = (int)p.win_len.size(); s.row_window = p.row_window; s.lds_bytes = p.lds_bytes;
    s.n_windows_lds = 0;
    for (int v : p.win_len) s.n_windows_lds += v > 0;
    s.window_nnz_frac = window_frac;
    s.x_window_hybrid = p.win_hybrid ? 1 : 0;
    if (p.windowed) { const int wpw = std::min(16, p.row_window / kMedRows); s.n_workgroups = ceil_div(s.n_long_pieces, wpw) + ceil_div(s.n_windows, 8) * 8 + (win_fold_tiles(s.n_windows, s.n_short_tiles) ? 0 : ceil_div(s.n_short_tiles, wpw)); }
    return DASP_OK;
}

template <class T> static int finish(Build<T> &bld)
{
    Plan &p = bld.p;
    if (bld.dev && !bld.meta_only) {
        PackMeta meta;
        meta.ridL = &bld.ridL; meta.startL = &bld.startL; meta.ridM = &bld.ridM; meta.lenM = &bld.lenM;
        for (int g = 0; g < kNumShortGroups; ++g) meta.glist[g] = bld.glist[g];
        if (int rc = devpack_all(p, *bld.dev, meta)) return rc;
        bld.lap("device pack");
    }
    if (bld.meta_only) {
        p.cnt_long = p.cnt_reg = p.cnt_irr = p.cnt_short = 0;
        p.piece_ptr.clear(); p.piece_dst.clear(); p.multi_ptr.clear(); p.multi_dst.clear(); p.piece_c16.clear(); p.long_base.clear(); p.long_cid16.clear(); p.cnt_long_chunks = 0;
        p.med_ptr.clear(); p.irr_ptr.clear();
        for (int g = 0; g < kNumShortGroups; ++g) { p.grp[g].tiles = 0; p.grp[g].tile0 = 0; p.grp[g].elem_off = 0; }
    }
    p.stats.pre_ms = bld.lap.ms();
    return DASP_OK;
}

template <class T> static int run_stages(Build<T> &bld)
{
    int (*const stages[])(Build<T> &) = {classify_rows<T>, sort_medium_by_length<T>, measure_reference<T>, assign_slots<T>, decide_windows<T>, medium_rows_as_pieces<T>,
                                         pack_long<T>, split_medium_chunks<T>, pack_medium<T>, pack_short<T>, fill_stats<T>, finish<T>};
    for (auto stage : stages)
        if (int rc = stage(bld)) return rc;
    return DASP_OK;
}

template <class T> static int build_dasp(Plan &p, const int *rp, const int *ci, const T *val, const DevCsr *dev, bool meta_only)
{
    Build<T> bld(p, rp, ci, val, dev, meta_only);
    if (!row_ptr_ends_ok(rp, bld.m, bld.nnz)) return DASP_ERR_ARG;
    bld.lap("validate");
    return run_stages(bld);
}

template <class T> static int build_form(Plan &p, const int *rp, const int *ci_in, const T *val_in, const DevCsr *dev_in)
{
    Build<T> bld(p, rp, ci_in, val_in, dev_in, false);
    if (int rc = validate_csr(bld)) return rc;
    SortedCsr<T> sorted;
    struct MapSrcReset { Plan &q; ~MapSrcReset() { q.map_src = nullptr; } } map_src_reset{p};
    if (int rc = sort_columns(bld, sorted)) return rc;
    int scattered = 0;
    const int P = decide_panels(p, bld.probe(), &scattered);
    if (P < 0) return P;
    if (decide_two_phase(p, rp, scattered)) {
        if (int rc = build_dasp<T>(p, rp, bld.ci, bld.val, nullptr, true)) return rc;
        bld.lap("whole-matrix meta");
        int rc2;
        if (!bld.dev) { rc2 = hybrid_then_tp(bld, bld.ci, bld.val); bld.lap("two-phase streams"); if (rc2 != kTpDeclined) return rc2; }
        else {
            rc2 = devpack_forms_enabled() ? hybrid_then_tp_device(bld) : kDevNoScratch;
            if (rc2 == kDevNoScratch) {
                rc2 = hybrid_then_tp_fetched(bld);
                if (rc2 == DASP_OK) return devpack_finish_panels(p);
            }
            if (rc2 == DASP_OK) return DASP_OK;
            if (rc2 != kTpDeclined) return rc2;
        }
    }
    if (P >= 2) return build_panels<T>(p, rp, bld.ci, bld.val, P, bld.dev);
    return run_stages(bld);
}

static int decide_panels(const Plan &p, const CsrProbe &probe, int *scattered)
{
    const int *rp = probe.rp;
    if (scattered) *scattered = 0;
    const int want = p.opt.col_panels;
    if (want > 64) { set_error("col_panels must be <= 64"); return DASP_ERR_ARG; }
    if (!p.dst_map.empty()) return 1;
    if (want == 1 || want < 0) return 1;
    if (want >= 2) return p.nnz > 0 && p.m > 0 ? want : 1;
    const long long xlen = p.opt.n_parts > 0 ? (long long)p.opt.n_parts * p.opt.part_stride : (long long)p.n;
    const long long vb = p.geo.vbytes, xbytes = xlen * vb;
// ... 313 lines not shown
```

dasp_amd/csrc/plan.hpp:

```cpp
#pragma once

#include <cstddef>
#include <cstdint>
#include <memory>
#include <string>
#include <utility>
#include <vector>

#include "../../include/dasp_amd.h"

namespace dasp {

template <class T>
struct NoInit : std::allocator<T> {
    template <class U> struct rebind { using other = NoInit<U>; };
    NoInit() = default;
    template <class U> NoInit(const NoInit<U> &) {}
    template <class U> void construct(U *p) noexcept { ::new (static_cast<void *>(p)) U; }
    template <class U, class... A> void construct(U *p, A &&...a) { ::new (static_cast<void *>(p)) U(std::forward<A>(a)...); }
};
template <class T> using raw_vector = std::vector<T, NoInit<T>>;

constexpr int kWave = 64;
constexpr long long kStreamBytes = 256ll << 20;
constexpr int kWavesPerWG = 4;

#ifndef DASP_SHOT16
#define DASP_SHOT16 4
#endif
constexpr int kMedBatch64 = 4, kMedShot64 = 8, kMedBatch16 = 2, kMedShot16 = DASP_SHOT16;
#if defined(__HIPCC__)
__host__ __device__
#endif
inline int med_npair(int nc, int nt, int vbytes, int mode)
{
    if (mode == 0) return 0;
    const int batch = vbytes == 8 ? kMedBatch64 : kMedBatch16, shot = vbytes == 8 ? kMedShot64 : kMedShot16;
    return nc + nt > shot ? nc / batch * batch : (vbytes == 2 || (mode == 2 && nt == 0) ? nc & ~1 : 0);
}
#if defined(__HIPCC__)
__host__ __device__
#endif
inline size_t med_cid8_index(int q, int lane, int ch, bool oneshot = false)
{
    return oneshot ? (size_t)(q & ~1) * ch + 2 * (size_t)lane + (q & 1) : (size_t)(q & ~3) * ch + 4 * (size_t)lane + (q & 3);
}
#if defined(__HIPCC__)
__host__ __device__
#endif
inline bool med_oneshot64(int nc, int nt) { return nc + nt <= kMedShot64; }
#if defined(__HIPCC__)
__host__ __device__
#endif
inline int med_n8(int narrow_in_paired_region, int nc, int nt) { return nc + nt > kMedShot64 ? narrow_in_paired_region / kMedBatch64 * kMedBatch64 : narrow_in_paired_region / 2 * 2; }
#if defined(__HIPCC__)
__host__ __device__
#endif
inline size_t med_elem_index(int npair, int c, int lane, int j, int vpl, int ch)
{
    return c < npair ? (size_t)(c & ~1) * ch + (size_t)vpl * (2 * lane + (c & 1)) + j : (size_t)c * ch + (size_t)vpl * lane + j;
}
#ifndef DASP_SHORT_TPW
#define DASP_SHORT_TPW 4
#endif
constexpr int kShortTpw = DASP_SHORT_TPW;
constexpr int kMedRows = 16;
constexpr int kLongAlign = 4;
constexpr int kLong16MinChunks = 4;
constexpr unsigned short kLongPad16 = 0xFFFFu;
constexpr int kSlabMaxLen = 32;
constexpr int kNumShortGroups = 5 + (kSlabMaxLen - 4);

struct Geometry {
    int vbytes;
    int med_k;
    int chunk;
    int short_rows;
};
inline Geometry geometry_for(int precision)
{
    return precision == 64 ? Geometry{8, 4, 64, 128} : Geometry{2, 16, 256, 256};
}

struct SlotMap {
    int split;
    int base[2], grp[2], off[2];
    int slot(int t) const
    {
        const int p = t < split ? 0 : 1;
        const int u = p ? t - split : t;
        return grp[p] ? base[p] + (u / grp[p]) * 2 * grp[p] + off[p] + u % grp[p] : base[p] + u;
    }
};

struct ShortGroup {
    int len = 0;
    int count = 0;
    int tiles = 0;
    int tile0 = 0;
    long long elem_off = 0;
    SlotMap map{};
    int seg = 0;
    int rpt = 0;
// ... 115 lines not shown
    int row_window = 0, lds_bytes = 0;
    std::vector<int> med_dst, win_cmin, win_len;

    ShortGroup grp[kNumShortGroups];
    raw_vector<char> short_val;
    raw_vector<int> short_cid;

    size_t cnt_long = 0, cnt_reg = 0, cnt_irr = 0, cnt_short = 0;
    size_t cnt_long_chunks = 0;

    std::vector<std::unique_ptr<dasp_plan>> panels;
    std::vector<int> panel_bounds;
    bool panel = false;
    const int *scan_order = nullptr;
    std::vector<int> dst_map;

    int rt_max = 0;
    std::vector<int> rt_ptr;
    std::vector<uint16_t> rt_start;
    std::vector<uint64_t> rt_mask;
    raw_vector<char> rt_val;
    raw_vector<int> rt_cid;
    size_t cnt_rt = 0;

    LongCB lcb;

    bool two_phase = false;
    TwoPhase tp;
    bool tp_exact = false;
    bool hub_exact = false;
    bool f32_vectors = false;

    bool value_map = false;
    std::vector<uint32_t> long_map, med_map, irr_map, short_map, rt_map;
    const uint32_t *map_src = nullptr;
    bool loaded = false;

    bool host_dropped = false;
    long long csr_fetch_bytes = 0;
    mutable long long sh_paired_bytes = 0, sh_shared_bytes = 0;
    mutable bool sh_known = false;
    bool sh_in_use = false;
    DevicePlan *dev = nullptr;

    ~Plan();
};

struct SharedIds {
    std::vector<uint32_t> plane, table;
    long long paired_id_bytes = 0;
    long long shared_bytes = 0;
    int n_pipelined = 0;
};
bool shared_ids_qualify(const Plan &p);
bool derive_shared_ids(const Plan &p, SharedIds &out);

struct DevCsr { const int *rp, *ci; const void *val; const uint32_t *src = nullptr; };
struct PackMeta {
    const std::vector<int> *ridL = nullptr; const std::vector<long long> *startL = nullptr;
    const raw_vector<int> *ridM = nullptr, *lenM = nullptr;
    const std::vector<int> *glist[kNumShortGroups] = {};
};
int devpack_validate(const Plan &p, const DevCsr &d);
int devpack_window_spans(const Plan &p, const DevCsr &d, const raw_vector<int> &ridW, int R, int *lo, int *hi, long long *wnnz);
int devpack_line_scatter(const Plan &p, const DevCsr &d, const std::vector<int> &rows, long long *lines, long long *entries);
int devpack_row_coherence(const Plan &p, const DevCsr &d, const std::vector<int> &rows, int within, long long *near, long long *entries);
int devpack_chunk_spans(const Plan &p, const DevCsr &d, const raw_vector<int> &ridM, const raw_vector<int> &lenM,
                        const std::vector<int> &nchunks, int *k16, unsigned long long *narrow_mask);
int devpack_densest_spans(const Plan &p, const DevCsr &d, const raw_vector<int> &ridW, const raw_vector<int> &lenW, int R, const std::vector<int> &wlist,
                          long long cap_cols, int A, int *hmin, long long *hin);
int devpack_all(Plan &p, const DevCsr &d, const PackMeta &m);
int devpack_finish_panels(Plan &p);
int devpack_fetch_csr(const Plan &p, const DevCsr &d, int *ci, void *val);
struct DevTiles {
    const unsigned long long *keys = nullptr; const uint32_t *idx = nullptr; const int *start = nullptr;
    long long n = 0, bins = 0;
    std::vector<std::shared_ptr<void>> keep;
};
constexpr int kDevNoScratch = 2;
bool devpack_forms_enabled();
int devpack_tp_count(const Plan &p, const DevCsr &d, const int *rp, const unsigned char *skip, const std::vector<int> &pos_of_row, int n_cb, DevTiles &out, std::vector<int> &cnt);
int devpack_lcb_count(const Plan &p, const DevCsr &d, const int *rp, DevTiles &out, std::vector<int> &cnt);
int devpack_finish_two_phase(Plan &p, const DevCsr &d, const DevTiles &tp, const std::vector<long long> &off2, const std::vector<long long> &off1, const DevTiles &lcb);
int devpack_finish_panels_lcb(Plan &p, const DevCsr &d, const DevTiles &lcb);
void release_device(Plan &p);
int devpack_current_device();
void devpack_use_device(int device);
int devpack_gather_columns(const Plan &p, const DevCsr &d, const std::vector<long long> *idx, long long start, long long stride, long long count, std::vector<int> &out);
int devpack_panel_split(const Plan &p, const DevCsr &d, const std::vector<int> &bnd, int P, std::vector<std::vector<int>> &rpP_host,
                        std::vector<DevCsr> &out, std::vector<std::shared_ptr<void>> &keep);
int devpack_panel_split_masked(const Plan &p, const DevCsr &d, const std::vector<int> &bnd, int P, std::vector<std::vector<int>> &rpP_host,
                               std::vector<DevCsr> &out, std::vector<std::shared_ptr<void>> &keep, const unsigned char *mask);

struct DevRowTiles { void *val = nullptr; int *cid = nullptr; uint32_t *map = nullptr; };
int devpack_row_tiles(const Plan &p, DevCsr &panel, const std::vector<int> &rp_rest, const std::vector<int> &at, size_t cnt,
                      std::vector<std::shared_ptr<void>> &keep, DevRowTiles *out);
int devpack_place_row_tiles(Plan &q, const DevRowTiles &src);

int devpack_sort_columns(const Plan &p, const DevCsr &d, std::vector<std::shared_ptr<void>> &keep, DevCsr *out, int *did);

int build_plan(Plan &p, const int *rp, const int *ci, const void *val, const DevCsr *dev = nullptr);

int decide_two_phase(const Plan &p, const int *rp, int scattered);
constexpr int kWinLdsMax = 160 * 1024 - 256;
inline int win_fold_tiles(int n_windows, int n_short_tiles)
{
// ... 36 lines not shown
```

dasp_amd/csrc/planio.cpp:

```cpp
#include <algorithm>
#include <cstdio>
#include <cstring>
#include <string>

#include "plan.hpp"

namespace dasp {

namespace {
const char kPlanMagic[8] = {'D', 'A', 'S', 'P', 'P', 'L', 'N', '8'};

struct Writer {
    FILE *f; bool ok = true;
    void raw(const void *p, size_t n) { if (ok && n && std::fwrite(p, 1, n, f) != n) ok = false; }
    template <class V> void vec(const V &v) { long long b = (long long)(v.size() * sizeof(typename V::value_type)); raw(&b, 8); raw(v.data(), (size_t)b); }
};
struct Reader {
    FILE *f; long long left; bool ok = true;
    void raw(void *p, size_t n)
    {
        if (!ok || !n) return;
        if ((long long)n > left || std::fread(p, 1, n, f) != n) { ok = false; return; }
        left -= (long long)n;
    }
    template <class V> void vec(V &v)
    {
        long long b = -1; raw(&b, 8);
        if (!ok || b < 0 || b > left || b % (long long)sizeof(typename V::value_type)) { ok = false; return; }
        v.resize((size_t)b / sizeof(typename V::value_type));
        raw(v.data(), (size_t)b);
    }
};

template <class IO> void arrays(IO &io, Plan &p)
{
    io.vec(p.part_bounds); io.vec(p.order); io.vec(p.dst_map); io.vec(p.panel_bounds);
    io.vec(p.long_val); io.vec(p.long_cid); io.vec(p.long_cid16); io.vec(p.long_base); io.vec(p.piece_c16); io.vec(p.piece_ptr); io.vec(p.piece_dst); io.vec(p.multi_ptr); io.vec(p.multi_dst);
    io.vec(p.med_ptr); io.vec(p.med_val); io.vec(p.med_cid); io.vec(p.med_cid16); io.vec(p.med_cid8); io.vec(p.med_c8ptr); io.vec(p.med_korig); io.vec(p.med_base);
    io.vec(p.irr_ptr); io.vec(p.irr_val); io.vec(p.irr_cid);
    io.vec(p.med_dst); io.vec(p.win_cmin); io.vec(p.win_len);
    io.vec(p.short_val); io.vec(p.short_cid);
    io.vec(p.rt_ptr); io.vec(p.rt_start); io.vec(p.rt_mask); io.vec(p.rt_val); io.vec(p.rt_cid);
    io.vec(p.tp.rb_row0); io.vec(p.tp.rb_seg0); io.vec(p.tp.unit); io.vec(p.tp.dst); io.vec(p.tp.lcol); io.vec(p.tp.lrow); io.vec(p.tp.val);
    io.vec(p.lcb.row_dst); io.vec(p.lcb.row_id); io.vec(p.lcb.ptr); io.vec(p.lcb.unit); io.vec(p.lcb.lcol); io.vec(p.lcb.val);
}
}

static bool validate_plan(const Plan &p, int n_panels, bool is_panel, std::string &why)
{
    auto fail = [&](const char *w) { why = w; return false; };
    const Geometry geo = p.geo;
    const long long vb = geo.vbytes, CH = geo.chunk, SR = geo.short_rows;
    const long long m = p.m;
    if (p.m < 0 || p.n < 0 || p.nnz < 0) return fail("negative dimension");
    if (p.opt.y_order != DASP_Y_PERMUTED && p.opt.y_order != DASP_Y_NATURAL) return fail("y_order");
    if (p.opt.n_parts < 0 || p.opt.n_parts > (1 << 20) || (p.opt.n_parts > 0 && p.opt.part_stride <= 0)) return fail("column partition");
    if (p.opt.n_parts > 0) {
        if (p.part_bounds.size() != (size_t)p.opt.n_parts + 1 || p.part_bounds.front() != 0 || p.part_bounds.back() != p.n) return fail("part_bounds size / span");
        for (int g = 0; g < p.opt.n_parts; ++g)
            if (p.part_bounds[g + 1] < p.part_bounds[g] || p.part_bounds[g + 1] - p.part_bounds[g] > p.opt.part_stride) return fail("part_bounds not monotone or wider than part_stride");
    } else if (!p.part_bounds.empty()) return fail("part_bounds without n_parts");
    const long long xlen = p.opt.n_parts > 0 ? (long long)p.opt.n_parts * p.opt.part_stride : (long long)p.n;
    if (xlen >= (1ll << 31)) return fail("x length");
    if (p.order.size() != (size_t)m) return fail("order size");
    {
        std::vector<bool> seen((size_t)m, false);
        for (int v : p.order) {
            if ((unsigned)v >= (unsigned)m) return fail("order_rid entry out of range");
            if (seen[(size_t)v]) return fail("order_rid is not a permutation: two writers for one y index in natural order");
            seen[(size_t)v] = true;
        }
    }
    if (!p.dst_map.empty()) {
        if (p.dst_map.size() != (size_t)m) return fail("dst_map size");
        for (int v : p.dst_map) if ((unsigned)v >= (unsigned)m) return fail("dst_map entry out of range");
    }
    if (p.stats.rowA != p.m || p.stats.colA != p.n || p.stats.nnzA != p.nnz || p.stats.precision != p.precision) return fail("stats header");
    if (p.stats.row_long < 0 || p.n_mfma_rows < 0 || p.n_mfma_rows > p.stats.row_block || (long long)p.stats.row_long + p.stats.row_block > m) return fail("category counters");
    if (n_panels == 0 && (p.med_slot0 < p.stats.row_long || (long long)p.med_slot0 + p.n_mfma_rows > (long long)p.stats.row_long + p.stats.row_block)) return fail("med_slot0");
    if (p.panel_bounds.size() != 2 * (size_t)n_panels) return fail("panel_bounds size");
    if (p.two_phase) {
        if (n_panels > 0 || is_panel) return fail("two-phase plan with column panels");
        if (p.cnt_long || p.cnt_reg || p.cnt_irr || p.cnt_short || p.cnt_rt || !p.med_ptr.empty() || !p.irr_ptr.empty() || !p.piece_ptr.empty()) return fail("two-phase plan holds packed DASP arrays");
        if (!validate_two_phase(p, why)) return false;
        if (!validate_long_cb(p, 0, why)) return false;
        long long have = 0;
        for (uint16_t r : p.tp.lrow) have += r != kTpPadRow;
        for (uint16_t c : p.lcb.lcol) have += c != kLcbPadCol;
        if (have != p.nnz) return fail("the two-phase streams and the column-blocked hub rows do not add up to nnzA");
        return true;
    }
    if (!p.tp.dst.empty() || !p.tp.lcol.empty() || !p.tp.lrow.empty() || !p.tp.val.empty() || !p.tp.unit.empty() || !p.tp.rb_row0.empty() || !p.tp.rb_seg0.empty()) return fail("two-phase streams in a plan that is not two-phase");
    if (n_panels == 0 && (p.lcb.n_rows() > 0 || !p.lcb.ptr.empty() || !p.lcb.lcol.empty() || !p.lcb.val.empty() || !p.lcb.unit.empty() || !p.lcb.row_id.empty())) return fail("column-blocked long rows outside a column-panel plan");
    if (n_panels > 0) {
        if (p.cnt_long || p.cnt_reg || p.cnt_irr || p.cnt_short || !p.med_ptr.empty() || !p.irr_ptr.empty() || !p.piece_ptr.empty()) return fail("panel parent holds packed arrays");
        for (int k = 0; k < n_panels; ++k)
            if (p.panel_bounds[2 * k] < 0 || p.panel_bounds[2 * k + 1] < p.panel_bounds[2 * k] || p.panel_bounds[2 * k + 1] > xlen) return fail("panel_bounds range");
        return validate_long_cb(p, n_panels, why);
    }
    auto cid_ok = [&](const raw_vector<int> &c) { for (int v : c) if (v < -1 || v >= xlen) return false; return true; };
    auto mono = [](const std::vector<int> &a) { if (a.empty() || a[0] != 0) return false; for (size_t i = 1; i < a.size(); ++i) if (a[i] < a[i - 1]) return false; return true; };
    if (p.long_val.size() != p.cnt_long * (size_t)vb || p.long_cid.size() != p.cnt_long) return fail("long arrays");
    if (p.piece_ptr.size() != p.piece_dst.size() + 1 || !mono(p.piece_ptr) || (size_t)p.piece_ptr.back() != p.cnt_long) return fail("piece_ptr");
    if (p.multi_ptr.size() != p.multi_dst.size() + 1 || !mono(p.multi_ptr)) return fail("multi_ptr");
    const long long n_partial = p.multi_ptr.back();
    for (int d : p.piece_dst) if (d >= 0 ? d >= m : (long long)~d >= n_partial) return fail("piece_dst out of range");
    for (int d : p.multi_dst) if ((unsigned)d >= (unsigned)m) return fail("multi_dst out of range");
    for (size_t i = 0; i + 1 < p.piece_ptr.size(); ++i) if (p.piece_ptr[i] % kLongAlign) return fail("piece_ptr alignment");
    if (!cid_ok(p.long_cid)) return fail("long_cid out of range");
    {
        const size_t np = p.piece_dst.size();
        if (p.piece_c16.size() != 2 * np || p.long_cid16.size() != p.cnt_long) return fail("long_cid16 / piece_c16 sizes");
        long long chunks = 0;
        for (size_t q = 0; q < np; ++q) {
            if (p.piece_c16[2 * q] != chunks || (unsigned)p.piece_c16[2 * q + 1] > 1u) return fail("piece_c16");
            chunks += (p.piece_ptr[q + 1] - p.piece_ptr[q] + CH - 1) / CH;
        }
        if ((long long)p.long_base.size() != chunks || (long long)p.cnt_long_chunks != chunks) return fail("long_base size");
        for (size_t q = 0; q < np; ++q) {
            const bool narrow = p.piece_c16[2 * q + 1] != 0;
            if (narrow && p.piece_ptr[q + 1] - p.piece_ptr[q] < kLong16MinChunks * CH) return fail("narrow piece shorter than four chunks");
            for (long long e = p.piece_ptr[q], c = p.piece_c16[2 * q]; e < p.piece_ptr[q + 1]; e += CH, ++c) {
                const int b = p.long_base[(size_t)c];
                if (b < 0 || b >= std::max<long long>(xlen, 1)) return fail("long_base out of range");
                for (long long j = e; j < std::min<long long>(e + CH, p.piece_ptr[q + 1]); ++j) {
                    const int col = p.long_cid[(size_t)j]; const unsigned o = p.long_cid16[(size_t)j];
                    if (narrow ? (col < 0 ? o != kLongPad16 : (o == kLongPad16 || b + (int)o != col)) : o != 0) return fail("long_cid16 does not match long_cid");
                }
            }
        }
    }
    const long long nb = (p.n_mfma_rows + kMedRows - 1) / kMedRows;
    if (p.med_ptr.size() != (size_t)nb + 1 || !mono(p.med_ptr) || p.stats.n_med_blocks != nb) return fail("med_ptr size / n_med_blocks");
    if ((size_t)p.med_ptr.back() * (size_t)CH != p.cnt_reg || p.med_val.size() != p.cnt_reg * (size_t)vb) return fail("regular tiles");
    if (p.cid16 ? (p.med_cid16.size() + p.med_cid8.size() != p.cnt_reg || p.med_cid8.size() != p.cnt_reg8 || !p.med_cid.empty() ||
                   p.med_base.size() != (size_t)p.med_ptr.back() || p.med_korig.size() != p.med_base.size() || p.med_c8ptr.size() != (size_t)nb + 1)
                : (p.med_cid.size() != p.cnt_reg || !p.med_cid16.empty() || !p.med_cid8.empty() || !p.med_base.empty() || !p.med_c8ptr.empty() || !p.med_korig.empty()))
        return fail("medium column ids");
    auto npair_of = [&](long long b) {
        const long long r0 = b * kMedRows, K = CH / kMedRows;
        return med_npair((int)(p.med_ptr[(size_t)b + 1] - p.med_ptr[(size_t)b]), (int)((p.irr_ptr[(size_t)r0 + 1] - p.irr_ptr[(size_t)r0] + K - 1) / K), (int)vb, p.pair_mode);
    };
    auto oneshot_of = [&](long long b) {
        const long long r0 = b * kMedRows, K = CH / kMedRows;
        return vb == 8 && med_oneshot64((int)(p.med_ptr[(size_t)b + 1] - p.med_ptr[(size_t)b]), (int)((p.irr_ptr[(size_t)r0 + 1] - p.irr_ptr[(size_t)r0] + K - 1) / K));
    };
    if (p.irr_ptr.size() != (size_t)p.n_mfma_rows + 1 || !mono(p.irr_ptr) || (size_t)p.irr_ptr.back() != p.cnt_irr) return fail("irr_ptr");
    if (p.irr_val.size() != p.cnt_irr * (size_t)vb || p.irr_cid.size() != p.cnt_irr) return fail("irregular arrays");
    if (!cid_ok(p.irr_cid) || !cid_ok(p.med_cid)) return fail("medium column id out of range");
    if (p.cid16) {
        if (!mono(p.med_c8ptr) || (size_t)p.med_c8ptr.back() * (size_t)CH != p.cnt_reg8) return fail("med_c8ptr");
        for (long long b = 0; b < nb; ++b) {
            const int nc = p.med_ptr[(size_t)b + 1] - p.med_ptr[(size_t)b], n8 = p.med_c8ptr[(size_t)b + 1] - p.med_c8ptr[(size_t)b], npair = npair_of(b);
            const bool one = med_oneshot64(nc, (p.irr_ptr[(size_t)b * kMedRows + 1] - p.irr_ptr[(size_t)b * kMedRows] + 3) / 4);
            if (n8 < 0 || n8 > npair || n8 % (one ? 2 : kMedBatch64) || (n8 && vb != 8))
                return fail("med_c8ptr: one-byte ids come in whole batches (pipelined) / pairs (one-shot) of an f64 block's paired region");
            std::vector<char> seen((size_t)nc, 0);
            for (int q = 0; q < nc; ++q) {
                const unsigned k = (unsigned)p.med_korig[(size_t)p.med_ptr[(size_t)b] + (size_t)q];
                if (k >= (unsigned)nc || seen[k] || (q >= npair && (int)k != q)) return fail("med_korig is not a permutation of its block's paired region");
                seen[k] = 1;
            }
        }
    }
    const int vpl = (int)(CH / 64);
    auto cid_at = [&](long long b, long long c, long long e) -> long long {
        const long long c0 = p.med_ptr[(size_t)b];
        const int npair = npair_of(b), q = (int)(c - c0), lane = (int)(e / vpl), j = (int)(e % vpl);
        if (!p.cid16) return p.med_cid[(size_t)c0 * (size_t)CH + med_elem_index(npair, q, lane, j, vpl, (int)CH)];
        const long long c8 = p.med_c8ptr[(size_t)b];
        const int n8 = (int)(p.med_c8ptr[(size_t)b + 1] - c8);
        if (q < n8) { const unsigned o = p.med_cid8[(size_t)c8 * (size_t)CH + med_cid8_index(q, lane, (int)CH, oneshot_of(b))]; return o == 0xFFu ? -1 : (long long)p.med_base[(size_t)c] + o; }
        const unsigned o = p.med_cid16[(size_t)(c0 - c8) * (size_t)CH + med_elem_index(npair - n8, q - n8, lane, j, vpl, (int)CH)];
        return o == 0xFFFFu ? -1 : (long long)p.med_base[(size_t)c] + o;
    };
    if (p.cid16)
        for (long long b = 0; b < nb; ++b)
            for (long long c = p.med_ptr[(size_t)b]; c < p.med_ptr[(size_t)b + 1]; ++c) {
                const long long base = p.med_base[(size_t)c];
                if (base < 0 || base >= std::max<long long>(xlen, 1)) return fail("med_base out of range");
                for (long long e = 0; e < CH; ++e) if (cid_at(b, c, e) >= xlen) return fail("16-bit column id out of range");
            }
    if (p.lds_bytes < 0 || p.lds_bytes > kWinLdsMax) return fail("lds_bytes");
    if (p.windowed) {
        if (p.row_window < 64 || p.row_window > 1024 || p.row_window % kMedRows) return fail("row_window");
        const long long nW = (p.n_mfma_rows + p.row_window - 1) / p.row_window;
        if (p.win_len.size() != (size_t)nW || p.win_cmin.size() != (size_t)nW || p.med_dst.size() != (size_t)p.n_mfma_rows) return fail("window tables");
        for (int d : p.med_dst) if ((unsigned)d >= (unsigned)m) return fail("med_dst out of range");
        const long long A = 16 / vb, bpw = p.row_window / kMedRows;
        for (long long w = 0; w < nW; ++w) {
            const long long len = p.win_len[(size_t)w], c0 = p.win_cmin[(size_t)w];
            if (len < 0 || c0 < 0 || len * vb > p.lds_bytes || c0 % A || (len > 0 && c0 + len > xlen)) return fail("window span");
            if (len == 0 || p.win_hybrid) continue;
            for (long long b = w * bpw; b < std::min(nb, (w + 1) * bpw); ++b) {
                for (long long c = p.med_ptr[(size_t)b]; c < p.med_ptr[(size_t)b + 1]; ++c)
                    for (long long e = 0; e < CH; ++e) {
                        const long long col = cid_at(b, c, e);
                        if (col < 0) continue;
                        if (col < c0 || col >= c0 + len) return fail("windowed column id outside its LDS span");
                    }
                for (long long r = b * kMedRows; r < std::min<long long>(p.n_mfma_rows, (b + 1) * kMedRows); ++r)
                    for (int t = p.irr_ptr[(size_t)r]; t < p.irr_ptr[(size_t)r + 1]; ++t) { const int col = p.irr_cid[(size_t)t]; if (col >= 0 && (col < c0 || col >= c0 + len)) return fail("windowed tail id outside its LDS span"); }
            }
        }
    } else if (!p.med_dst.empty() || !p.win_len.empty() || !p.win_cmin.empty()) return fail("window tables without windows");
    if (p.short_val.size() != p.cnt_short * (size_t)vb || p.short_cid.size() != p.cnt_short || !cid_ok(p.short_cid)) return fail("short arrays");
    long long off = 0, tile0 = 0;
// ... 55 lines not shown
        for (int d : p.piece_dst) if (d >= 0 && !claim(d)) return fail("two writers for one y index (piece_dst)");
        for (int d : p.multi_dst) if (!claim(d)) return fail("two writers for one y index (multi_dst)");
        for (long long r = 0; r < p.n_mfma_rows; ++r)
            if (!claim(p.windowed ? (long long)p.med_dst[(size_t)r] : ydst((long long)p.med_slot0 + r))) return fail("two writers for one y index (medium rows)");
        for (int g = 0; g < kNumShortGroups; ++g) {
            if (is_panel && p.grp[g].len == 0) continue;
            for (int t = 0; t < p.grp[g].count; ++t)
                if (!claim(ydst(g < 5 ? (long long)p.grp[g].map.slot(t) : (long long)p.grp[g].map.base[0] + t))) return fail("two writers for one y index (short rows / slabs)");
        }
    }
    return true;
}

static void write_plan(Writer &w, Plan &p)
{
    const int hdr[25] = {p.precision, p.m, p.n, p.nnz, p.opt.y_order, p.windowed ? 1 : 0, p.row_window, p.lds_bytes, p.cid16 ? 1 : 0,
                         p.opt.n_parts, p.opt.part_stride, p.opt.stream_policy, (int)p.panels.size(), p.n_mfma_rows, p.win_hybrid ? 1 : 0, p.med_slot0, p.pair_mode, p.win_rel16 ? 1 : 0, p.rt_max,
                         p.two_phase ? 1 : 0, p.tp.cb, p.tp.rb_max, p.lcb.cb, p.lcb.n_cb, p.lcb.h};
    w.raw(hdr, sizeof hdr); w.raw(&p.stats, sizeof p.stats); w.raw(p.grp, sizeof p.grp);
    arrays(w, p);
    for (auto &h : p.panels) write_plan(w, h->impl);
}

static bool read_plan(Reader &r, Plan &p, int depth, std::string &r_why)
{
    int hdr[25];
    r.raw(hdr, sizeof hdr);
    if (!r.ok || (hdr[0] != 64 && hdr[0] != 16) || hdr[12] < 0 || hdr[12] > 64 || (depth > 0 && hdr[12] != 0)) return false;
    p.precision = hdr[0]; p.geo = geometry_for(p.precision);
    p.m = hdr[1]; p.n = hdr[2]; p.nnz = hdr[3];
    dasp_options_default(&p.opt);
    p.opt.y_order = hdr[4]; p.windowed = hdr[5] != 0; p.row_window = hdr[6]; p.lds_bytes = hdr[7]; p.cid16 = hdr[8] != 0;
    p.opt.n_parts = hdr[9]; p.opt.part_stride = hdr[10]; p.opt.stream_policy = hdr[11]; p.n_mfma_rows = hdr[13]; p.win_hybrid = hdr[14] != 0; p.med_slot0 = hdr[15]; p.pair_mode = hdr[16]; p.win_rel16 = hdr[17] != 0; p.rt_max = hdr[18];
    if (p.pair_mode < 0 || p.pair_mode > 2 || (p.windowed && p.pair_mode)) return false;
    p.two_phase = hdr[19] != 0; p.tp.cb = hdr[20]; p.tp.rb_max = hdr[21];
    p.lcb.cb = hdr[22]; p.lcb.n_cb = hdr[23]; p.lcb.h = hdr[24];
    if (p.two_phase && (depth > 0 || hdr[12] != 0)) return false;
    r.raw(&p.stats, sizeof p.stats); r.raw(p.grp, sizeof p.grp);
    arrays(r, p);
    if (!r.ok) return false;
    p.tp.segments = p.tp.dst.size();
    p.lcb.elems = p.lcb.lcol.size();
    p.opt.two_phase = p.two_phase ? 1 : -1; p.opt.tp_col_block = p.tp.cb; p.opt.tp_row_block = p.tp.rb_max;
    p.opt.part_bounds = p.part_bounds.empty() ? nullptr : p.part_bounds.data();
    const size_t vb = (size_t)p.geo.vbytes;
    const int np = hdr[12];
    bool sane = p.m >= 0 && p.order.size() == (size_t)p.m && p.stats.rowA == p.m && p.stats.precision == p.precision &&
                (p.dst_map.empty() || p.dst_map.size() == (size_t)p.m) && p.panel_bounds.size() == 2 * (size_t)np &&
                p.long_val.size() == p.long_cid.size() * vb && p.irr_val.size() == p.irr_cid.size() * vb &&
                p.short_val.size() == p.short_cid.size() * vb &&
                (p.cid16 ? p.med_val.size() == (p.med_cid16.size() + p.med_cid8.size()) * vb : p.med_val.size() == p.med_cid.size() * vb);
    if (np == 0 && !p.two_phase)
        sane = sane && p.piece_ptr.size() == p.piece_dst.size() + 1 && p.irr_ptr.size() == (size_t)p.n_mfma_rows + 1 &&
               p.n_mfma_rows >= 0 && p.n_mfma_rows <= p.stats.row_block && (!p.windowed || p.med_dst.size() == (size_t)p.n_mfma_rows);
    if (!sane) return false;
    p.cnt_long = p.long_cid.size(); p.cnt_irr = p.irr_cid.size(); p.cnt_short = p.short_cid.size();
    p.cnt_long_chunks = p.long_base.size();
    p.cnt_reg = p.cid16 ? p.med_cid16.size() + p.med_cid8.size() : p.med_cid.size();
    p.cnt_reg8 = p.med_cid8.size();
    p.cnt_rt = p.rt_cid.size();
    p.host_dropped = false;
    p.loaded = true;
    p.panel = depth > 0;
    if (!validate_plan(p, np, depth > 0, r_why)) return false;
    if (p.two_phase) p.tp.max_row = tp_longest_row(p.tp);
    p.lcb.max_row = lcb_longest_row(p.lcb);
    p.opt.col_panels = np > 0 ? np : 1;
    for (int k = 0; k < np; ++k) {
        std::unique_ptr<dasp_plan> h(new dasp_plan());
        if (!read_plan(r, h->impl, depth + 1, r_why) || h->impl.m != p.m || h->impl.precision != p.precision) return false;
        p.panels.push_back(std::move(h));
    }
    if (np > 0) {
        long long have = 0;
        for (const auto &h : p.panels) have += (long long)h->impl.nnz + (long long)h->impl.cnt_rt;
        for (uint16_t c : p.lcb.lcol) have += c != kLcbPadCol;
        if (have != p.nnz) { r_why = "the panels and the column-blocked long rows do not add up to nnzA"; return false; }
    }
    return true;
}

int save_plan(Plan &p, const char *path)
{
    if (!path) return DASP_ERR_ARG;
    if (p.host_dropped) { set_error("host arrays were dropped: nothing to save"); return DASP_ERR_STATE; }
    FILE *f = std::fopen(path, "wb");
    if (!f) { set_error(std::string("cannot create ") + path); return DASP_ERR_OPEN; }
    Writer w{f};
    w.raw(kPlanMagic, 8);
    const int abi[3] = {(int)sizeof(dasp_stats_t), kNumShortGroups, (int)sizeof(ShortGroup)};
    w.raw(abi, sizeof abi);
    write_plan(w, p);
    const bool ok = (std::fclose(f) == 0) && w.ok;
    if (!ok) { set_error(std::string("short write to ") + path); return DASP_ERR_OPEN; }
    return DASP_OK;
}

int load_plan(Plan &p, const char *path)
{
    if (!path) return DASP_ERR_ARG;
    FILE *f = std::fopen(path, "rb");
    if (!f) { set_error(std::string("cannot open ") + path); return DASP_ERR_OPEN; }
    std::fseek(f, 0, SEEK_END);
    const long long size = std::ftell(f);
    std::fseek(f, 0, SEEK_SET);
    Reader r{f, size < 0 ? 0 : size};
    char magic[8];
// ... 17 lines not shown
```

dasp_amd/csrc/sharedids.cpp:

```cpp
#include <cstring>

#include "plan.hpp"

namespace dasp {

bool shared_ids_qualify(const Plan &p)
{
    if (p.precision != 64 || !p.cid16 || p.windowed || p.two_phase || !p.panels.empty() || p.panel || p.host_dropped) return false;
    const size_t nb = p.med_ptr.empty() ? 0 : p.med_ptr.size() - 1;
    if (nb == 0 || p.med_c8ptr.size() != nb + 1 || p.irr_ptr.size() < 2) return false;
    return p.med_cid8.size() == p.cnt_reg8 && p.med_cid16.size() == p.cnt_reg - p.cnt_reg8 && p.cnt_reg > 0;
}

bool derive_shared_ids(const Plan &p, SharedIds &out)
{
    out = SharedIds();
    if (!shared_ids_qualify(p)) return false;
    constexpr int CH = 64, K = 4;
    const size_t nb = p.med_ptr.size() - 1;
    out.table.assign(4 * nb, 0u);
    const unsigned char *c8 = p.med_cid8.data();
    const unsigned char *c16 = reinterpret_cast<const unsigned char *>(p.med_cid16.data());
    std::vector<const unsigned char *> slot;
    for (size_t b = 0; b < nb; ++b) {
        const int c0 = p.med_ptr[b], nc = p.med_ptr[b + 1] - c0;
        const size_t r0 = b * (size_t)kMedRows;
        const int nt = r0 + 1 < p.irr_ptr.size() ? (p.irr_ptr[r0 + 1] - p.irr_ptr[r0] + K - 1) / K : 0;
        if (med_oneshot64(nc, nt)) continue;
        const int npair = med_npair(nc, nt, 8, p.pair_mode);
        if (npair <= 0) continue;
        const int q0 = p.med_c8ptr[b], n8 = p.med_c8ptr[b + 1] - q0;
        slot.clear();
        for (int i = 0; i < n8; i += kMedBatch64) slot.push_back(c8 + (size_t)(q0 + i) * CH);
        for (int i = n8; i < npair; i += 2) slot.push_back(c16 + 2 * (size_t)(c0 - q0 - n8 + i) * CH);
        auto same = [&](int r, int q) {
            for (const unsigned char *s : slot)
                for (int kq = 0; kq < 4; ++kq)
                    if (std::memcmp(s + 4 * (r + 16 * kq), s + 4 * (q + 16 * kq), 4) != 0) return false;
            return true;
        };
        int rep[kMedRows], rank[kMedRows], L = 0;
        for (int r = 0; r < kMedRows; ++r) {
            int g = 0;
            while (g < L && !same(r, rep[g])) ++g;
            if (g == L) rep[L++] = r;
            rank[r] = g;
        }
        unsigned long long ranks = 0;
        for (int r = 0; r < kMedRows; ++r) ranks |= (unsigned long long)rank[r] << (4 * r);
        const size_t at = out.plane.size();
        out.plane.resize(at + slot.size() * 4 * (size_t)L);
        uint32_t *dst = out.plane.data() + at;
        for (const unsigned char *s : slot)
            for (int kq = 0; kq < 4; ++kq)
                for (int g = 0; g < L; ++g) std::memcpy(dst++, s + 4 * (rep[g] + 16 * kq), 4);
        out.table[4 * b] = (uint32_t)ranks; out.table[4 * b + 1] = (uint32_t)(ranks >> 32);
        out.table[4 * b + 2] = (uint32_t)(at / 4); out.table[4 * b + 3] = (uint32_t)L;
        out.paired_id_bytes += (long long)slot.size() * 4 * CH;
        ++out.n_pipelined;
        if (at / 4 > 0xFFFFFFFFull) { out = SharedIds(); return false; }
    }
    if (out.n_pipelined == 0) { out = SharedIds(); return false; }
    out.shared_bytes = (long long)out.plane.size() * 4 + (long long)out.table.size() * 4;
    return true;
}

}
```

dasp_amd/csrc/upload.cpp:

```cpp
#include <hip/hip_runtime_api.h>

#include <algorithm>
#include <chrono>
#include <cmath>
#include <cstdio>
#include <cstdlib>
#include <cstring>
#include <string>
#include <type_traits>
#include <vector>

#include "plan.hpp"
#include "device.hpp"

namespace dasp {

#define HIP_TRY(expr)                                                                          \
    do {                                                                                       \
        hipError_t e_ = (expr);                                                                \
        if (e_ != hipSuccess) {                                                                \
            set_error(std::string(#expr) + ": " + hipGetErrorString(e_));                      \
            return e_ == hipErrorNoDevice ? DASP_ERR_NO_DEVICE : DASP_ERR_HIP;                 \
        }                                                                                      \
    } while (0)
// ... 54 lines not shown
    HIP_TRY(hipMemcpy(base + o.p, L.ptr.data(), L.ptr.size() * 4, hipMemcpyHostToDevice));
    HIP_TRY(hipMemcpy(base + o.u, L.unit.data(), L.unit.size() * 4, hipMemcpyHostToDevice));
    HIP_TRY(hipMemcpy(base + o.d, L.row_dst.data(), L.row_dst.size() * 4, hipMemcpyHostToDevice));
    HIP_TRY(hipMemset(base + o.s, 0, std::max<size_t>((size_t)L.n_cb * (size_t)L.n_rows() * 8, 16)));
    LcbDev &q = d->lcb;
    q.val = base + o.v; q.lcol = (const unsigned short *)(base + o.c); q.ptr = (const int *)(base + o.p); q.unit = (const int *)(base + o.u);
    q.row_dst = (const int *)(base + o.d); q.partial = base + o.s;
    q.n_units = L.n_units(); q.n_rows = L.n_rows(); q.n_cb = L.n_cb; q.cb = L.cb; q.xlen = p.n;
    q.xpart = nullptr; q.xsteps = 1;
    for (int u = 0; u < L.n_units(); ++u) q.xsteps = std::max(q.xsteps, (L.ptr[(size_t)L.unit[3 * (size_t)u + 2]] - L.ptr[(size_t)L.unit[3 * (size_t)u + 1]]) / kLcbStep);
    if (has_exact_hub_kernels(p)) {
        const size_t bytes = std::max<size_t>((size_t)L.n_cb * (size_t)L.n_rows() * 20, 16);
        HIP_TRY(hipMalloc(&d->lcb_xpart, bytes));
        HIP_TRY(hipMemset(d->lcb_xpart, 0, bytes));
        q.xpart = d->lcb_xpart;
    }
    if (int rc = tp_kernels_allow_lds()) return rc;
    return DASP_OK;
}

static bool long16_rule(const Plan &p, long long *narrow_elems)
{
    bool on = false;
    long long narrow = 0;
    if (!p.windowed && p.cnt_reg8 == 0 && p.piece_c16.size() == 2 * p.piece_dst.size() && !p.piece_dst.empty()) {
        for (size_t q = 0; q < p.piece_dst.size(); ++q) if (p.piece_c16[2 * q + 1]) narrow += p.piece_ptr[q + 1] - p.piece_ptr[q];
        on = narrow * 20 >= (long long)p.nnz && narrow > 0;
        if (const char *e = std::getenv("DASP_LONG16")) on = std::atoi(e) != 0;
    }
    if (narrow_elems) *narrow_elems = narrow;
    return on;
}
void choose_long16(Plan &p)
{
    DevicePlan *d = p.dev;
    if (!d) return;
    d->long16 = long16_rule(p, nullptr);
}

long long shared_ids_net_saving(const Plan &p, const SharedIds &s, bool long16)
{
    long long narrow = 0;
    (void)long16_rule(p, &narrow);
    return s.paired_id_bytes - s.shared_bytes - (long16 ? 2 * narrow : 0);
}
static bool seven_waves_rule(const Plan &p)
{
    bool on = false;
    if (p.precision == 64 && !p.windowed && p.med_ptr.size() > 1 && p.irr_ptr.size() > 1) {
        long long one = 0, all = 0;
        const int K = p.geo.med_k, nbk = (int)p.med_ptr.size() - 1;
        for (int b = 0; b < nbk; ++b) {
            const int nc = p.med_ptr[(size_t)b + 1] - p.med_ptr[(size_t)b], r0 = b * kMedRows;
            const int nt = (p.irr_ptr[(size_t)r0 + 1] - p.irr_ptr[(size_t)r0] + K - 1) / K;
            all += nc + nt;
            if (med_oneshot64(nc, nt)) one += nc + nt;
        }
        on = all > 0 && one * 10 >= all * 7 && p.stats.data_X > (64ll << 20);
        if (const char *e = std::getenv("DASP_SEVEN_WAVES")) on = std::atoi(e) != 0;
    }
    return on;
}
static int share_ids_env() { const char *e = std::getenv("DASP_SHARE_IDS"); return e ? (std::atoi(e) != 0 ? 1 : 0) : -1; }
static bool shared_ids_rule(const Plan &p, const SharedIds &s)
{
    if (seven_waves_rule(p)) return false;
    const int env = share_ids_env();
    if (env >= 0) return env == 1;
    return p.stats.data_X > kStreamBytes && shared_ids_net_saving(p, s, long16_rule(p, nullptr)) * 100 >= 3 * p.stats.data_X;
}

void release_device(Plan &p)
{
    if (p.dev) {
        value_map_free(p.dev); if (p.dev->arena) (void)hipFree(p.dev->arena); if (p.dev->lcb_xpart) (void)hipFree(p.dev->lcb_xpart);
        if (p.dev->wide_xs) (void)hipFree(p.dev->wide_xs);
        if (p.dev->wide_part) (void)hipFree(p.dev->wide_part);
        if (p.dev->dargs) (void)hipFree(p.dev->dargs); std::free(p.dev->args_sent); delete p.dev; p.dev = nullptr;
    }
    p.f32_vectors = false;
}

int set_f32_vectors_device(Plan &p, int on)
{
    DevicePlan *d = p.dev;
    if (!d || !d->arena) { set_error("plan not uploaded"); return DASP_ERR_STATE; }
    if (!on) {
        if (!p.f32_vectors) return DASP_OK;
        HIP_TRY(hipDeviceSynchronize());
        p.f32_vectors = false;
        if (d->wide_xs) (void)hipFree(d->wide_xs);
        if (d->wide_part) (void)hipFree(d->wide_part);
        d->wide_xs = d->wide_part = nullptr;
        return DASP_OK;
    }
    if (p.f32_vectors) return DASP_OK;
    const size_t xs_bytes = std::max<size_t>(p.tp.segments * (size_t)kTpSeg * 4, 16);
    const size_t part_bytes = p.lcb.n_rows() > 0 ? std::max<size_t>((size_t)p.lcb.n_cb * (size_t)p.lcb.n_rows() * 8, 16) : 0;
    void *xs = nullptr, *part = nullptr;
    auto make = [&]() -> hipError_t {
        if (hipError_t e = hipMalloc(&xs, xs_bytes)) return e;
        if (hipError_t e = hipMemset(xs, 0, xs_bytes)) return e;
        if (part_bytes) {
            if (hipError_t e = hipMalloc(&part, part_bytes)) return e;
            if (hipError_t e = hipMemset(part, 0, part_bytes)) return e;
        }
        return hipDeviceSynchronize();
// ... 62 lines not shown
        q.lcol = (const unsigned short *)(base + o_lc); q.dst = (const int *)(base + o_dst); q.unit = (const int *)(base + o_un);
        q.val = base + o_v; q.lrow = (const unsigned short *)(base + o_lr); q.xs = base + o_xs;
        q.rb_row0 = (const int *)(base + o_r0); q.rb_seg0 = (const int *)(base + o_s0);
        q.n_units = t.n_units(); q.n_rb = t.n_rb(); q.cb = t.cb; q.rb_max = t.rb_max; q.xlen = p.n; q.m = p.m;
        d->nt = true;
        if (lcb) if (int rc = upload_long_cb(p, d, lo)) { release_device(p); return rc; }
        return tp_kernels_allow_lds();
    }

    std::vector<ShortDev> groups(kNumShortGroups);
    for (int g = 0; g < kNumShortGroups; ++g) {
        groups[g].len = p.grp[g].len; groups[g].count = p.grp[g].count; groups[g].tiles = p.grp[g].tiles;
        groups[g].tile0 = p.grp[g].tile0; groups[g].elem_off = p.grp[g].elem_off; groups[g].map = p.grp[g].map;
        groups[g].seg = p.grp[g].seg; groups[g].rpt = p.grp[g].rpt;
    }
    const bool natural = p.opt.y_order == DASP_Y_NATURAL;
    const size_t part_bytes = (size_t)std::max<size_t>(1, p.multi_ptr.empty() ? 0 : (size_t)p.multi_ptr.back()) * 8;

    struct Item { const void *src; size_t bytes; size_t off; };
    std::vector<Item> items;
    size_t total = 0;
    auto add = [&](const void *src, size_t bytes) {
        size_t off = total;
        items.push_back({src, bytes, off});
        total += (bytes + 255) & ~size_t(255);
        if (bytes == 0) total += 256;
        return off;
    };
    auto src_of = [](const auto &v) -> const void * { return v.empty() ? nullptr : v.data(); };
    const size_t vbytes = (size_t)p.geo.vbytes;
    const size_t o_lv = add(src_of(p.long_val), p.cnt_long * vbytes);
    const size_t o_lc = add(src_of(p.long_cid), p.cnt_long * 4);
    const size_t o_lc16 = add(src_of(p.long_cid16), p.cnt_long * 2);
    const size_t o_lb = add(src_of(p.long_base), p.cnt_long_chunks * 4);
    const size_t o_pc16 = add(p.piece_c16.data(), p.piece_c16.size() * 4);
    const size_t o_pp = add(p.piece_ptr.data(), p.piece_ptr.size() * 4);
    const size_t o_pd = add(p.piece_dst.data(), p.piece_dst.size() * 4);
    const size_t o_mp = add(p.multi_ptr.data(), p.multi_ptr.size() * 4);
    const size_t o_md = add(p.multi_dst.data(), p.multi_dst.size() * 4);
    const size_t o_part = add(nullptr, part_bytes);
    const size_t o_mptr = add(p.med_ptr.data(), p.med_ptr.size() * 4);
    const size_t o_mv = add(src_of(p.med_val), p.cnt_reg * vbytes);
    const size_t o_mc = add(src_of(p.med_cid), p.cid16 ? 0 : p.cnt_reg * 4);
    const size_t o_mc16 = add(src_of(p.med_cid16), p.cid16 ? (p.cnt_reg - p.cnt_reg8) * 2 : 0);
    const size_t o_mc8 = add(src_of(p.med_cid8), p.cnt_reg8);
    const size_t o_c8p = add(p.med_c8ptr.data(), p.med_c8ptr.size() * 4);
    const size_t o_mb = add(src_of(p.med_base), p.cid16 ? (size_t)p.med_ptr.back() * 4 : 0);
    const size_t o_ip = add(p.irr_ptr.data(), p.irr_ptr.size() * 4);
    std::vector<int> med_nt((size_t)std::max(p.stats.n_med_blocks, 0), 0);
    {
        const int TK = p.precision == 64 ? 4 : 16;
        for (size_t b = 0; b < med_nt.size(); ++b) {
            const size_t r0 = b * (size_t)kMedRows;
            if (r0 + 1 < p.irr_ptr.size()) med_nt[b] = (p.irr_ptr[r0 + 1] - p.irr_ptr[r0] + TK - 1) / TK;
        }
    }
    const size_t o_mnt = add(med_nt.data(), med_nt.size() * 4);
    const size_t o_iv = add(src_of(p.irr_val), p.cnt_irr * vbytes);
    const size_t o_ic = add(src_of(p.irr_cid), p.cnt_irr * 4);
    const size_t o_mdst = add(p.med_dst.data(), p.med_dst.size() * 4);
    const size_t o_wc = add(p.win_cmin.data(), p.win_cmin.size() * 4);
    const size_t o_wl = add(p.win_len.data(), p.win_len.size() * 4);
    const size_t o_sv = add(src_of(p.short_val), p.cnt_short * vbytes);
    const size_t o_sc = add(src_of(p.short_cid), p.cnt_short * 4);
    const size_t o_g = add(groups.data(), groups.size() * sizeof(ShortDev));
    const size_t o_rv = add(src_of(p.rt_val), p.cnt_rt * vbytes);
    const size_t o_rc = add(src_of(p.rt_cid), p.cnt_rt * 4);
    const size_t o_rp = add(p.rt_ptr.data(), p.rt_ptr.size() * 4);
    const size_t o_rs = add(p.rt_start.data(), p.rt_start.size() * 2);
    const size_t o_rm = add(p.rt_mask.data(), p.rt_mask.size() * 8);
    std::vector<int> ord_mapped;
    if (natural && !p.dst_map.empty()) { ord_mapped.resize(p.order.size()); for (size_t i = 0; i < p.order.size(); ++i) ord_mapped[i] = p.dst_map[(size_t)p.order[i]]; }
    const size_t o_ord = add(natural ? (ord_mapped.empty() ? p.order.data() : ord_mapped.data()) : nullptr, natural ? p.order.size() * 4 : 0);
    SharedIds sh;
    size_t o_shp = 0, o_sht = 0;
    d->shared_ids = false;
    p.sh_in_use = false;
    if (share_ids_env() != 0 && (p.stats.data_X > kStreamBytes || share_ids_env() == 1)) {
        const bool have = derive_shared_ids(p, sh);
        p.sh_paired_bytes = sh.paired_id_bytes; p.sh_shared_bytes = sh.shared_bytes; p.sh_known = true;
        p.sh_in_use = d->shared_ids = have && shared_ids_rule(p, sh);
        if (d->shared_ids) { o_shp = add(sh.plane.data(), sh.plane.size() * 4); o_sht = add(sh.table.data(), sh.table.size() * 4); }
    }

    HIP_TRY(hipMalloc(&d->arena, total));
    d->arena_bytes = total;
    if (std::getenv("DASP_VERBOSE")) std::fprintf(stderr, "[dasp upload] arena %p + %zu bytes\n", d->arena, total);
    char *base = static_cast<char *>(d->arena);
    for (const Item &it : items)
        if (it.src && it.bytes) HIP_TRY(hipMemcpy(base + it.off, it.src, it.bytes, hipMemcpyHostToDevice));

    d->map.long_val = o_lv; d->map.long_cid = o_lc; d->map.med_val = o_mv; d->map.med_cid = o_mc; d->map.med_cid16 = o_mc16; d->map.med_cid8 = o_mc8;
    d->map.med_base = o_mb; d->map.irr_val = o_iv; d->map.irr_cid = o_ic; d->map.short_val = o_sv; d->map.short_cid = o_sc;
    d->map.rt_val = o_rv; d->map.rt_cid = o_rc; d->map.long_cid16 = o_lc16; d->map.long_base = o_lb; d->map.piece_c16 = o_pc16;
    DevArgs &a = d->args;
    a.long_val = base + o_lv; a.long_cid = (const int *)(base + o_lc);
    a.long_cid16 = (const unsigned short *)(base + o_lc16); a.long_base = (const int *)(base + o_lb); a.piece_c16 = (const int *)(base + o_pc16);
    a.piece_ptr = (const int *)(base + o_pp); a.piece_dst = (const int *)(base + o_pd);
    a.multi_ptr = (const int *)(base + o_mp); a.multi_dst = (const int *)(base + o_md);
    a.partial = base + o_part;
    a.n_pieces = (int)p.piece_dst.size(); a.n_multi = (int)p.multi_dst.size();
    a.med_ptr = (const int *)(base + o_mptr); a.med_val = base + o_mv; a.med_cid = (const int *)(base + o_mc);
    a.irr_ptr = (const int *)(base + o_ip); a.med_nt = (const int *)(base + o_mnt); a.irr_val = base + o_iv; a.irr_cid = (const int *)(base + o_ic);
    a.n_blocks = p.stats.n_med_blocks; a.row_block = p.n_mfma_rows; a.row_long = p.med_slot0;
    for (int g = 0; g < kNumShortGroups; ++g) a.grp_tile0[g] = p.grp[g].tile0;
    a.short_val = base + o_sv; a.short_cid = (const int *)(base + o_sc); a.groups = (const ShortDev *)(base + o_g);
    a.n_short_tiles = p.stats.n_short_tiles;
// ... 186 lines not shown
```

include/dasp_amd.h:

```cpp
#ifndef DASP_AMD_H
#define DASP_AMD_H

#include <stddef.h>
#include <stdint.h>

#ifdef __cplusplus
extern "C" {
#endif

typedef enum dasp_status {
    DASP_OK = 0,
    DASP_ERR_OPEN = -1,
    DASP_ERR_BANNER = -2,
    DASP_ERR_SIZE = -4,
    DASP_ERR_ENTRY = -5,
    DASP_ERR_ARG = -10,
    DASP_ERR_NOMEM = -11,
    DASP_ERR_NO_DEVICE = -20,
    DASP_ERR_HIP = -21,
    DASP_ERR_STATE = -22
} dasp_status;

const char *dasp_last_error(void);
const char *dasp_version(void);

int dasp_mmio_allinone_f64(int *m, int *n, int *nnz, int *isSymmetric,
                           int **csrRowPtr, int **csrColIdx, double **csrVal, const char *filename);
int dasp_mmio_allinone_f16(int *m, int *n, int *nnz, int *isSymmetric,
                           int **csrRowPtr, int **csrColIdx, uint16_t **csrVal, const char *filename);
void dasp_free(void *p);

int dasp_csr_save(const char *path, int precision, int m, int n, int nnz, int isSymmetric,
                  const int *csrRowPtr, const int *csrColIdx, const void *csrVal);
int dasp_csr_load(const char *path, int precision, int *m, int *n, int *nnz, int *isSymmetric,
                  int **csrRowPtr, int **csrColIdx, void **csrVal);

typedef struct dasp_plan dasp_plan_t;

typedef enum { DASP_F64 = 64, DASP_F16 = 16 } dasp_precision;
typedef enum {
    DASP_Y_PERMUTED = 0,
    DASP_Y_NATURAL = 1
} dasp_y_order;

typedef struct dasp_options {
    double threshold;
    int block_longest;
    int y_order;
    int long_piece;
    int host_threads;
    int n_parts;
    const int *part_bounds;
    int part_stride;
    int x_window;
    int row_window;
    int cid16;
    int stream_policy;
    int col_panels;
    int slab_max_len;
    int x_window_hybrid;
    int piece_min_len;
    int chunk_pairs;
    int cid8;
    int short_seg;
    int row_tile_max;
    int sort_columns;
    int two_phase;
    int tp_col_block, tp_row_block;
    int long_cb;
    int value_map;
    int tp_exact;
} dasp_options_t;

void dasp_options_default(dasp_options_t *opt);

typedef struct dasp_stats {
    int precision, rowA, colA, nnzA;
    int short_row_1, common_13, short_row_3, short_row_4, short_row_2, row_long, row_block, row_zero;
    int nnz_short, nnz_long, origin_nnz_reg, nnz_irreg;
    int rowloop;
    long long fill0_nnz_short, fill0_nnz_long, fill0_nnz_reg;
    double rate_fill0;
    long long data_X;
    long long data_origin1;
    int n_med_blocks, n_long_pieces, n_long_multi, n_short_tiles, n_workgroups;
    double pre_ms;
    int x_window_on, n_windows, n_windows_lds, lds_bytes, row_window;
    double window_nnz_frac;
    int cid16_on;
    int n_col_panels;
    int x_window_hybrid;
    int med_rows_as_pieces;
    int chunk_pairs;
    int cid8_chunks;
    int short_seg;
    int row_tile_max;
    int n_row_tiles;
    long long row_tile_nnz;
    int two_phase;
    int tp_col_block, tp_row_blocks, tp_units;
    long long tp_segments;
    int tp_seg_elems;
    int lcb_rows, lcb_col_block, lcb_units;
    long long lcb_elems;
    long long ref_fill0_nnz_short, ref_fill0_nnz_long, ref_fill0_nnz_reg, ref_data_X;
    int ref_nnz_irreg, ref_origin_nnz_reg, ref_blocknum, ref_warp_number;
    double ref_rate_fill0;
} dasp_stats_t;

int dasp_plan_create(dasp_plan_t **plan, int precision, int rowA, int colA, int nnzA,
                     const int *csrRowPtr, const int *csrColIdx, const void *csrVal,
                     const dasp_options_t *opt );
int dasp_plan_create_device(dasp_plan_t **plan, int precision, int rowA, int colA, int nnzA,
                            const int *dRowPtr, const int *dColIdx, const void *dVal, const dasp_options_t *opt);
int dasp_plan_tune_placement(dasp_plan_t *plan, int trials, const void *dX, void *dY, double *ms_first, double *ms_kept);
int dasp_plan_download_array(dasp_plan_t *plan, const char *name, void *dst, size_t bytes);
void dasp_plan_destroy(dasp_plan_t *plan);

int dasp_plan_save(dasp_plan_t *plan, const char *path);
int dasp_plan_load(dasp_plan_t **plan, const char *path);

const int *dasp_plan_order(const dasp_plan_t *plan);
int dasp_plan_stats(const dasp_plan_t *plan, dasp_stats_t *out);
int dasp_plan_y_order(const dasp_plan_t *plan);
long long dasp_plan_x_len(const dasp_plan_t *plan);

int dasp_plan_panel_count(const dasp_plan_t *plan);
dasp_plan_t *dasp_plan_panel(dasp_plan_t *plan, int k);
int dasp_plan_panel_range(const dasp_plan_t *plan, int k, int *col_begin, int *col_end);

long long dasp_plan_host_array(const dasp_plan_t *plan, const char *name, const void **ptr, int *elem_bytes);

int dasp_plan_upload(dasp_plan_t *plan);
int dasp_plan_drop_host(dasp_plan_t *plan);

int dasp_plan_update_values(dasp_plan_t *plan, const void *dVal, void *stream);
int dasp_plan_update_values_host(dasp_plan_t *plan, const void *csrVal);
long long dasp_plan_value_map_slots(const dasp_plan_t *plan);
long long dasp_plan_csr_fetch_bytes(const dasp_plan_t *plan);

int dasp_plan_shared_ids(const dasp_plan_t *plan, long long *paired_id_bytes, long long *shared_bytes, int *in_use);
long long dasp_plan_shared_ids_export(const dasp_plan_t *plan, const char *what, void *dst, size_t bytes);

int dasp_plan_set_stream_policy(dasp_plan_t *plan, int policy);

int dasp_plan_set_tp_exact(dasp_plan_t *plan, int on);
int dasp_plan_tp_exact(const dasp_plan_t *plan);
int dasp_plan_set_hub_exact(dasp_plan_t *plan, int on);
int dasp_plan_hub_exact(const dasp_plan_t *plan);
int dasp_tp_exact_dot_f16(const uint16_t *a, const uint16_t *x, long long n, int accumulate, uint16_t y_in, uint16_t *y_out);

int dasp_plan_spmv(dasp_plan_t *plan, const void *dX, void *dY, void *stream);
int dasp_plan_spmv_acc(dasp_plan_t *plan, const void *dX, void *dY, void *stream);

int dasp_plan_set_f32_vectors(dasp_plan_t *plan, int on);
int dasp_plan_f32_vectors(const dasp_plan_t *plan);
int dasp_plan_spmv_f32(dasp_plan_t *plan, const float *dX, float *dY, void *stream);
int dasp_plan_spmv_acc_f32(dasp_plan_t *plan, const float *dX, float *dY, void *stream);

int dasp_plan_time(dasp_plan_t *plan, const void *dX, void *dY, void *stream, int warmup, int iters,
                   double *wall_ms_per_iter, double *event_ms_per_iter);

int dasp_plan_time_each(dasp_plan_t *plan, const void *dX, void *dY, void *stream, int warmup, int iters, float *ms_each);

int dasp_plan_time_graph(dasp_plan_t *plan, const void *dX, void *dY, void *stream, int warmup, int iters, int batch,
                         double *wall_ms_per_iter, double *event_ms_per_iter);

int dasp_spmv_all_f64(const char *filename, const double *csrValA, const int *csrRowPtrA,
                      const int *csrColIdxA, const double *X_val, double *Y_val, int *order_rid,
                      int rowA, int colA, int nnzA, int NUM, double threshold, int block_longest);
int dasp_spmv_all_f16(const char *filename, const uint16_t *csrValA, const int *csrRowPtrA,
                      const int *csrColIdxA, const uint16_t *X_val, uint16_t *Y_val, int *order_rid,
                      int rowA, int colA, int nnzA, int NUM, double threshold, int block_longest);

typedef struct dasp_mg_plan dasp_mg_plan_t;
enum { DASP_MG_ID_BYTES = 128 };

typedef struct dasp_mg_info {
    int precision, n_gpus, rank, rowA, colA;
    int row_begin, row_end;
    int stride;
    long long nnz_own, nnz_other;
    int overlap, has_comm, square;
    int stream_memops;
    int fused_step;
    int exchange;
} dasp_mg_info_t;

int dasp_partition_rows(int rowA, const int *csrRowPtr, int n_parts, int *bounds);

int dasp_mg_unique_id(void *id);

int dasp_mg_plan_create(dasp_mg_plan_t **mg, int precision, int rowA, int colA, int n_gpus, int rank, const int *row_bounds,
                        const int *csrRowPtr, const int *csrColIdx, const void *csrVal, const dasp_options_t *opt, int overlap);
void dasp_mg_destroy(dasp_mg_plan_t *mg);
// ... 38 lines not shown
```

Measured before the change: 1282 GFLOP/s.

## Store single-piece long rows as MFMA medium blocks instead of long pieces

Adds a plan stage that can fold long rows that fit in one piece into the medium-row MFMA block path, prepending them to the medium row list. The stage is gated by a heuristic that checks regular-fill fraction, batch count and sampled row coherence. The irregular-tail count per block becomes the max over the block's 16 rows instead of the first row's, and this is updated in the kernel, planner, validator and upload. The aim is to drop the separate long-row kernel and its reduction overhead, at the cost of extra padding and a heavier planning step.

```diff
diff --git a/dasp_amd/_lib.py b/dasp_amd/_lib.py
--- a/dasp_amd/_lib.py
+++ b/dasp_amd/_lib.py
@@ -34,8 +34,25 @@
     def tp_exact(self, v):
         self._tp_exact_cell().value = int(v)
 
+    C_SIZE = 128
+
+    def __new__(cls, *args, **kwargs):
+        return cls.from_buffer(bytearray(cls.C_SIZE))
+
+    def _long_blocks_cell(self):
+        return C.c_int.from_address(C.addressof(self) + Options.value_map.offset + 2 * C.sizeof(C.c_int))
+
+    @property
+    def long_blocks(self):
+        return self._long_blocks_cell().value
+
+    @long_blocks.setter
+    def long_blocks(self, v):
+        self._long_blocks_cell().value = int(v)
+
 
 assert Options.value_map.offset + 2 * C.sizeof(C.c_int) <= C.sizeof(Options), "dasp_options_t::tp_exact must lie inside the Python mirror of the struct"
+assert Options.value_map.offset + 3 * C.sizeof(C.c_int) <= Options.C_SIZE and C.sizeof(Options) <= Options.C_SIZE, "dasp_options_t::long_blocks must lie inside an instance's buffer"
 
 
 class Stats(C.Structure):
@@ -147,6 +164,8 @@
         L.dasp_plan_shared_ids.argtypes = [vp, C.POINTER(C.c_longlong), C.POINTER(C.c_longlong), ip]
         L.dasp_plan_shared_ids_export.argtypes = [vp, C.c_char_p, vp, C.c_size_t]
         L.dasp_plan_shared_ids_export.restype = C.c_longlong
+    if hasattr(L, "dasp_plan_long_blocks"):
+        L.dasp_plan_long_blocks.argtypes = [vp, ip, C.POINTER(C.c_longlong)]
     L.dasp_plan_set_stream_policy.argtypes = [vp, C.c_int]
     if hasattr(L, "dasp_plan_set_tp_exact"):
         L.dasp_plan_set_tp_exact.argtypes = [vp, C.c_int]
@@ -220,7 +239,7 @@
 EXPORTS = (
     "dasp_last_error dasp_version dasp_mmio_allinone_f64 dasp_mmio_allinone_f16 dasp_free dasp_csr_save dasp_csr_load dasp_options_default "
     "dasp_plan_create dasp_plan_create_device dasp_plan_download_array dasp_plan_destroy dasp_plan_save dasp_plan_load dasp_plan_order dasp_plan_stats dasp_plan_y_order dasp_plan_x_len dasp_plan_panel_count dasp_plan_panel dasp_plan_panel_range dasp_plan_host_array dasp_plan_upload dasp_plan_tune_placement "
-    "dasp_plan_drop_host dasp_plan_update_values dasp_plan_update_values_host dasp_plan_value_map_slots dasp_plan_csr_fetch_bytes dasp_plan_shared_ids dasp_plan_shared_ids_export dasp_plan_set_stream_policy dasp_plan_set_tp_exact dasp_plan_tp_exact dasp_plan_set_hub_exact dasp_plan_hub_exact dasp_tp_exact_dot_f16 dasp_plan_spmv dasp_plan_spmv_acc dasp_plan_set_f32_vectors dasp_plan_f32_vectors dasp_plan_spmv_f32 dasp_plan_spmv_acc_f32 dasp_plan_time dasp_plan_time_each dasp_plan_time_graph dasp_spmv_all_f64 dasp_spmv_all_f16 dasp_partition_rows "
+    "dasp_plan_drop_host dasp_plan_update_values dasp_plan_update_values_host dasp_plan_value_map_slots dasp_plan_csr_fetch_bytes dasp_plan_shared_ids dasp_plan_shared_ids_export dasp_plan_long_blocks dasp_plan_set_stream_policy dasp_plan_set_tp_exact dasp_plan_tp_exact dasp_plan_set_hub_exact dasp_plan_hub_exact dasp_tp_exact_dot_f16 dasp_plan_spmv dasp_plan_spmv_acc dasp_plan_set_f32_vectors dasp_plan_f32_vectors dasp_plan_spmv_f32 dasp_plan_spmv_acc_f32 dasp_plan_time dasp_plan_time_each dasp_plan_time_graph dasp_spmv_all_f64 dasp_spmv_all_f16 dasp_partition_rows "
     "dasp_selftest_mfma dasp_synth_dims dasp_synth_generator dasp_synth_row_lengths dasp_synth_rows "
     "dasp_mg_unique_id dasp_mg_plan_create dasp_mg_destroy dasp_mg_upload dasp_mg_comm_init dasp_mg_set_x dasp_mg_spmv dasp_mg_product dasp_mg_allgather "
     "dasp_mg_wait dasp_mg_get_y dasp_mg_get_y_local dasp_mg_y_local dasp_mg_gathered dasp_mg_x dasp_mg_subplan dasp_mg_info dasp_mg_check dasp_mg_set_fused dasp_mg_set_fake_exchange "
diff --git a/dasp_amd/api.py b/dasp_amd/api.py
--- a/dasp_amd/api.py
+++ b/dasp_amd/api.py
@@ -72,7 +72,7 @@
     def __init__(self, csrRowPtr, csrColIdx, csrVal, colA, precision=64, threshold=0.75, block_longest=256,
                  y_order=Y_PERMUTED, long_piece=0, host_threads=0, part_bounds=None, part_stride=0, x_window=0, row_window=0, cid16=0, stream_policy=0,
                  col_panels=0, slab_max_len=0, x_window_hybrid=0, piece_min_len=0, chunk_pairs=0, cid8=0, short_seg=0, row_tile_max=0, sort_columns=0,
-                 two_phase=0, tp_col_block=0, tp_row_block=0, long_cb=0, value_map=0, tp_exact=0):
+                 two_phase=0, tp_col_block=0, tp_row_block=0, long_cb=0, value_map=0, tp_exact=0, long_blocks=0):
         L = _lib.lib()
         self.precision = precision
         dt = _dtype(precision)
@@ -88,7 +88,7 @@
         opt.col_panels, opt.slab_max_len, opt.x_window_hybrid, opt.piece_min_len = col_panels, slab_max_len, x_window_hybrid, piece_min_len
         opt.chunk_pairs, opt.cid8, opt.short_seg, opt.row_tile_max, opt.sort_columns = chunk_pairs, cid8, short_seg, row_tile_max, sort_columns
         opt.two_phase, opt.tp_col_block, opt.tp_row_block, opt.long_cb = two_phase, tp_col_block, tp_row_block, long_cb
-        opt.value_map, opt.tp_exact = value_map, tp_exact
+        opt.value_map, opt.tp_exact, opt.long_blocks = value_map, tp_exact, long_blocks
         self._pb = None
         if part_bounds is not None:
             self._pb = np.ascontiguousarray(part_bounds, np.int32)
@@ -104,7 +104,7 @@
     def from_device(cls, d_row_ptr, d_col_idx, d_val, rowA, colA, nnzA, precision=64, threshold=0.75, block_longest=256,
                     y_order=Y_PERMUTED, long_piece=0, part_bounds=None, part_stride=0, x_window=0, row_window=0, cid16=0, col_panels=0, slab_max_len=0,
                     x_window_hybrid=0, piece_min_len=0, chunk_pairs=0, cid8=0, short_seg=0, row_tile_max=0, sort_columns=0, two_phase=0, tp_col_block=0, tp_row_block=0, long_cb=0,
-                    value_map=0, tp_exact=0):
+                    value_map=0, tp_exact=0, long_blocks=0):
         L = _lib.lib()
         self = cls.__new__(cls)
         self.precision, self.rowA, self.colA, self.nnzA = precision, int(rowA), int(colA), int(nnzA)
@@ -115,7 +115,7 @@
         opt.slab_max_len, opt.x_window_hybrid, opt.piece_min_len = slab_max_len, x_window_hybrid, piece_min_len
         opt.chunk_pairs, opt.cid8, opt.short_seg, opt.row_tile_max, opt.sort_columns = chunk_pairs, cid8, short_seg, row_tile_max, sort_columns
         opt.two_phase, opt.tp_col_block, opt.tp_row_block, opt.long_cb = two_phase, tp_col_block, tp_row_block, long_cb
-        opt.value_map, opt.tp_exact = value_map, tp_exact
+        opt.value_map, opt.tp_exact, opt.long_blocks = value_map, tp_exact, long_blocks
         self._pb = None
         if part_bounds is not None:
             self._pb = np.ascontiguousarray(part_bounds, np.int32)
@@ -236,6 +236,13 @@
             _lib.check(rc)
         return {"available": bool(rc), "paired_id_bytes": int(pb.value), "shared_bytes": int(sb.value), "in_use": bool(use.value)}
 
+    def long_blocks(self):
+        rows, nnz = C.c_int(0), C.c_longlong(0)
+        rc = _lib.lib().dasp_plan_long_blocks(self._h, C.byref(rows), C.byref(nnz))
+        if rc < 0:
+            _lib.check(rc)
+        return int(rows.value), int(nnz.value)
+
     def shared_ids_export(self):
         out = []
         for what in (b"plane", b"table"):
diff --git a/dasp_amd/csrc/capi.cpp b/dasp_amd/csrc/capi.cpp
--- a/dasp_amd/csrc/capi.cpp
+++ b/dasp_amd/csrc/capi.cpp
@@ -101,6 +101,9 @@
     } else { p.opt.n_parts = 0; p.opt.part_bounds = nullptr; }
     if (p.opt.value_map != 0 && p.opt.value_map != 1) { set_error("value_map must be 0 or 1"); return DASP_ERR_ARG; }
     if (p.opt.tp_exact != 0 && p.opt.tp_exact != 1) { set_error("tp_exact must be 0 or 1"); return DASP_ERR_ARG; }
+    if (p.opt.long_blocks == kLongBlocksNever) p.opt.long_blocks = -1;
+    else if (const char *e = std::getenv("DASP_LONG_BLOCKS")) p.opt.long_blocks = std::atoi(e);
+    if (p.opt.long_blocks < -1 || p.opt.long_blocks > 1) { set_error("long_blocks must be -1, 0 or 1"); return DASP_ERR_ARG; }
     return DASP_OK;
 }
 
@@ -328,6 +331,16 @@
         if (shared_bytes) *shared_bytes = sb;
         return 1;
     });
+}
+
+int dasp_plan_long_blocks(const dasp_plan_t *plan, int *rows, long long *nnz)
+{
+    if (!plan) return DASP_ERR_ARG;
+    const Plan &p = plan->impl;
+    const bool on = long_rows_are_blocks(p);
+    if (rows) *rows = on ? p.stats.row_long : 0;
+    if (nnz) *nnz = on ? (long long)p.stats.nnz_long : 0;
+    return on ? 1 : 0;
 }
 
 long long dasp_plan_shared_ids_export(const dasp_plan_t *plan, const char *what, void *dst, size_t bytes)
diff --git a/dasp_amd/csrc/devpack.hip b/dasp_amd/csrc/devpack.hip
--- a/dasp_amd/csrc/devpack.hip
+++ b/dasp_amd/csrc/devpack.hip
@@ -165,11 +165,11 @@
     if (b >= nb) return;
     const int c0 = med_ptr[b], nc = med_ptr[b + 1] - c0;
     const int r0 = b * kMedRows;
-    const int nt_b = (irr_ptr[r0 + 1] - irr_ptr[r0] + K - 1) / K;
+    const int rr = lane & 15, kq = lane >> 4, r = r0 + rr;
+    const bool row_ok = r < nmed;
+    const int nt_b = (wave_max(row_ok ? irr_ptr[r + 1] - irr_ptr[r] : 0) + K - 1) / K;
     const int npair = med_npair(nc, nt_b, (int)sizeof(T), pair_mode);
     const bool oneshot = med_oneshot64(nc, nt_b);
-    const int rr = lane & 15, kq = lane >> 4, r = r0 + rr;
-    const bool row_ok = r < nmed;
     const int a0 = row_ok ? rp[ridM[r]] : 0, len = row_ok ? lenM[r] : 0;
     int n8 = 0, a8 = 0, a16 = 0; size_t e8 = 0, e16 = (size_t)c0 * CH;
     if constexpr (C16) { n8 = c8ptr[b + 1] - c8ptr[b]; e8 = (size_t)c8ptr[b] * CH; e16 = ((size_t)c0 - (size_t)c8ptr[b]) * CH; }
diff --git a/dasp_amd/csrc/multigpu.cpp b/dasp_amd/csrc/multigpu.cpp
--- a/dasp_amd/csrc/multigpu.cpp
+++ b/dasp_amd/csrc/multigpu.cpp
@@ -291,6 +291,7 @@
     opt.y_order = DASP_Y_NATURAL;
     opt.short_seg = -1;
     opt.two_phase = -1;
+    opt.long_blocks = kLongBlocksNever;
     opt.n_parts = 0; opt.part_bounds = nullptr; opt.part_stride = 0;
     opt.tp_exact = 0;
     opt.value_map = 0;
diff --git a/dasp_amd/csrc/plan.cpp b/dasp_amd/csrc/plan.cpp
--- a/dasp_amd/csrc/plan.cpp
+++ b/dasp_amd/csrc/plan.cpp
@@ -402,6 +402,7 @@
     double window_frac = 0.0;
     int nsp = 0;
     int rows_as_pieces = 0;
+    int long_block_rows = 0;
     std::vector<long long> startL;
     int nb = 0;
     long long n_reg = 0;
@@ -1108,17 +1109,14 @@
     return DASP_OK;
 }
 
-template <class T> static int pack_long(Build<T> &bld)
-{
-    Plan &p = bld.p;
+template <class T> static int piece_length(const Build<T> &bld)
+{
+    const Plan &p = bld.p;
     const Geometry &geo = bld.geo;
-    const int *rp = bld.rp, *ci = bld.ci;
-    const T *val = bld.val;
-    const Remap remap = bld.remap;
-    const int nnz = bld.nnz, threads = bld.threads, rows_as_pieces = bld.rows_as_pieces;
-    const bool f16 = bld.f16, pack = bld.pack;
+    const int *rp = bld.rp;
+    const int nnz = bld.nnz;
+    const bool f16 = bld.f16;
     const std::vector<int> &ridL = bld.ridL;
-    std::vector<long long> &startL = bld.startL;
     long long nnz_pieces = 0;
     for (int r : ridL) nnz_pieces += rp[r + 1] - rp[r];
     int piece = p.opt.long_piece > 0 ? p.opt.long_piece : 1024;
@@ -1130,7 +1128,81 @@
         const double rest_us = 4.0 + 3.0 + (double)nnz * (double)(geo.vbytes + 4) / 5.0e6;
         if ((nnz_pieces <= 2000000 && longest <= 16384 && chain_us <= rest_us) || longest <= one_piece) piece = std::max(piece, longest);
     }
-    piece = std::max(geo.chunk, ceil_div(piece, geo.chunk) * geo.chunk);
+    return std::max(geo.chunk, ceil_div(piece, geo.chunk) * geo.chunk);
+}
+
+template <class T> static int long_rows_as_blocks(Build<T> &bld)
+{
+    Plan &p = bld.p;
+    const Geometry &geo = bld.geo;
+    const int *rp = bld.rp;
+    const int row_long = bld.row_long, K = geo.med_k, CH = geo.chunk;
+    std::vector<int> &ridL = bld.ridL;
+    raw_vector<int> &ridM = bld.ridM, &lenM = bld.lenM, &ridM_in = bld.ridM_in;
+    bld.long_block_rows = 0;
+    const int want = p.opt.long_blocks;
+    if (want < 0 || row_long == 0 || bld.f16 || bld.meta_only || p.windowed || p.panel || !p.dst_map.empty() || bld.nsp != 0) return DASP_OK;
+    int longest = 0;
+    for (int r : ridL) longest = std::max(longest, rp[r + 1] - rp[r]);
+    const bool one_piece = ceil_div(longest, kLongAlign) * kLongAlign <= piece_length(bld);
+    if (want > 0 && !one_piece) { set_error("long_blocks = 1: a row is longer than one piece (long_piece); only single-piece long rows can be stored as blocks"); return DASP_ERR_ARG; }
+    if (!one_piece) return DASP_OK;
+    if (want == 0) {
+        if ((long long)bld.nnz * (geo.vbytes + 4) <= kStreamBytes) return DASP_OK;
+        const int nlb = ceil_div(row_long, kMedRows), mfma_rows = bld.mfma_rows;
+        long long reg = 0, all = 0;
+        for (int b = 0; b < nlb; ++b) {
+            int len[kMedRows], n = 0;
+            for (int i = b * kMedRows; i < (b + 1) * kMedRows && i < row_long + mfma_rows; ++i) len[n++] = i < row_long ? rp[ridL[(size_t)i] + 1] - rp[ridL[(size_t)i]] : lenM[(size_t)(i - row_long)];
+            int k = 0;
+            for (;; ++k) {
+                int fill = 0;
+                for (int i = 0; i < n; ++i) fill += std::min(K, std::max(0, len[i] - K * k));
+                if (!(fill >= p.opt.threshold * CH) || fill == 0) break;
+            }
+            for (int i = 0; i < n; ++i) { reg += std::min(len[i], K * k); all += len[i]; }
+        }
+        if ((double)reg < kLongBlocksRegular * (double)all) return DASP_OK;
+        const double est_us = (double)bld.nnz * (geo.vbytes + 4) / 5.0e6;
+        const int steps = ceil_div(longest, K), batches = steps <= kMedShot64 ? 1 : ceil_div(steps, kMedBatch64);
+        if (batches > std::max(2, (int)(0.25 * est_us / 0.8))) return DASP_OK;
+        std::vector<int> pairs;
+        int sampled = 0;
+        const int step = std::max(1, (row_long - 1) / 2048);
+        for (int i = 0; i + 1 < row_long; i += step, ++sampled)
+            if (rp[ridL[(size_t)i] + 1] - rp[ridL[(size_t)i]] == rp[ridL[(size_t)i + 1] + 1] - rp[ridL[(size_t)i + 1]]) { pairs.push_back(ridL[(size_t)i]); pairs.push_back(ridL[(size_t)i + 1]); }
+        if (sampled == 0 || (long long)pairs.size() < sampled) return DASP_OK;
+        long long near = 0, entries = 0;
+        if (int rc = bld.probe().row_coherence(pairs, 16, &near, &entries)) return rc;
+        if (entries == 0 || 2 * near < entries) return DASP_OK;
+    }
+    raw_vector<int> rid, len;
+    rid.reserve((size_t)row_long + ridM.size()); len.reserve((size_t)row_long + lenM.size());
+    for (int r : ridL) { rid.push_back(r); len.push_back(rp[r + 1] - rp[r]); }
+    rid.insert(rid.end(), ridM.begin(), ridM.end()); len.insert(len.end(), lenM.begin(), lenM.end());
+    ridM.swap(rid); lenM.swap(len);
+    (void)ridM_in;
+    ridL.clear();
+    bld.long_block_rows = row_long;
+    bld.rows_as_pieces = 0;
+    bld.mfma_rows += row_long;
+    p.med_slot0 = 0;
+    p.n_mfma_rows = bld.mfma_rows;
+    return DASP_OK;
+}
+
+template <class T> static int pack_long(Build<T> &bld)
+{
+    Plan &p = bld.p;
+    const Geometry &geo = bld.geo;
+    const int *rp = bld.rp, *ci = bld.ci;
+    const T *val = bld.val;
+    const Remap remap = bld.remap;
+    const int threads = bld.threads, rows_as_pieces = bld.rows_as_pieces;
+    const bool pack = bld.pack;
+    const std::vector<int> &ridL = bld.ridL;
+    std::vector<long long> &startL = bld.startL;
+    const int piece = piece_length(bld);
     {
         std::vector<long long> start((size_t)rows_as_pieces + 1, 0);
         for (int i = 0; i < rows_as_pieces; ++i) {
@@ -1257,7 +1329,9 @@
     if (try8 && p.cid16 && p.pair_mode > 0) {
         long long total8 = 0, total = 0;
         for (int b = 0; b < nb; ++b) {
-            const int nt = (p.irr_ptr[(size_t)b * kMedRows] + K - 1) / K, npair = med_npair(nchunks[b], nt, geo.vbytes, p.pair_mode);
+            int tail_b = 0;
+            for (int r = b * kMedRows, r1 = std::min(mfma_rows, r + kMedRows); r < r1; ++r) tail_b = std::max(tail_b, p.irr_ptr[(size_t)r]);
+            const int nt = (tail_b + K - 1) / K, npair = med_npair(nchunks[b], nt, geo.vbytes, p.pair_mode);
             const unsigned long long in = npair >= 64 ? ~0ull : ((1ull << npair) - 1);
             n8of[b] = p.opt.cid8 == 0 && med_oneshot64(nchunks[b], nt) ? 0 : med_n8(__builtin_popcountll(narrow_mask[(size_t)b] & in), nchunks[b], nt);
             total8 += n8of[b]; total += nchunks[b];
@@ -1333,7 +1407,7 @@
             const int nc = p.med_ptr[b + 1] - p.med_ptr[b];
             const size_t base = (size_t)p.med_ptr[b] * CH;
             const int r0 = (int)b * kMedRows, r1 = std::min(mfma_rows, r0 + kMedRows);
-            const int nt_b = (p.irr_ptr[r0 + 1] - p.irr_ptr[r0] + K - 1) / K;
+            const int nt_b = (med_block_tail(p.irr_ptr.data(), r0, mfma_rows) + K - 1) / K;
             const int npair = med_npair(nc, nt_b, geo.vbytes, p.pair_mode);
             const bool oneshot = med_oneshot64(nc, nt_b);
             const int n8 = p.cid16 ? p.med_c8ptr[b + 1] - p.med_c8ptr[b] : 0;
@@ -1484,8 +1558,9 @@
     for (int g = 0; g < kNumShortGroups; ++g) s.short_seg |= p.grp[g].seg;
     s.row_long = row_long; s.row_block = row_block; s.row_zero = nz0; s.med_rows_as_pieces = nsp; s.chunk_pairs = p.pair_mode; s.cid8_chunks = p.med_c8ptr.empty() ? 0 : p.med_c8ptr.back();
     s.nnz_short = nnz_short; s.nnz_long = (int)nnz_long; s.nnz_irreg = nnz_irreg;
-    s.origin_nnz_reg = nnz - nnz_irreg - (int)nnz_long - nnz_short;
-    s.rowloop = mfma_rows < 59990 ? 1 : (mfma_rows < 400000 ? 2 : 4);
+    s.origin_nnz_reg = nnz - nnz_irreg - (bld.long_block_rows > 0 ? 0 : (int)nnz_long) - nnz_short;
+    const int med_mfma_rows = mfma_rows - bld.long_block_rows;
+    s.rowloop = med_mfma_rows < 59990 ? 1 : (med_mfma_rows < 400000 ? 2 : 4);
     s.fill0_nnz_short = (long long)p.cnt_short;
     s.fill0_nnz_long = (long long)p.cnt_long;
     s.fill0_nnz_reg = n_reg;
@@ -1539,7 +1614,7 @@
 template <class T> static int run_stages(Build<T> &bld)
 {
     int (*const stages[])(Build<T> &) = {classify_rows<T>, sort_medium_by_length<T>, measure_reference<T>, assign_slots<T>, decide_windows<T>, medium_rows_as_pieces<T>,
-                                         pack_long<T>, split_medium_chunks<T>, pack_medium<T>, pack_short<T>, fill_stats<T>, finish<T>};
+                                         long_rows_as_blocks<T>, pack_long<T>, split_medium_chunks<T>, pack_medium<T>, pack_short<T>, fill_stats<T>, finish<T>};
     for (auto stage : stages)
         if (int rc = stage(bld)) return rc;
     return DASP_OK;
diff --git a/dasp_amd/csrc/plan.hpp b/dasp_amd/csrc/plan.hpp
--- a/dasp_amd/csrc/plan.hpp
+++ b/dasp_amd/csrc/plan.hpp
@@ -49,6 +49,12 @@
 __host__ __device__
 #endif
 inline bool med_oneshot64(int nc, int nt) { return nc + nt <= kMedShot64; }
+inline int med_block_tail(const int *irr_ptr, long long r0, long long nrows)
+{
+    int t = 0;
+    for (long long r = r0; r < nrows && r < r0 + 16; ++r) { const int v = irr_ptr[r + 1] - irr_ptr[r]; t = v > t ? v : t; }
+    return t;
+}
 #if defined(__HIPCC__)
 __host__ __device__
 #endif
@@ -270,6 +276,12 @@
     long long shared_bytes = 0;
     int n_pipelined = 0;
 };
+constexpr double kLongBlocksRegular = 0.9;
+constexpr int kLongBlocksNever = -2;
+inline bool long_rows_are_blocks(const Plan &p)
+{
+    return !p.two_phase && p.panels.empty() && p.stats.n_col_panels == 0 && p.stats.row_long > 0 && p.med_slot0 == 0 && p.n_mfma_rows >= p.stats.row_long && p.piece_dst.empty();
+}
 bool shared_ids_qualify(const Plan &p);
 bool derive_shared_ids(const Plan &p, SharedIds &out);
 
diff --git a/dasp_amd/csrc/planio.cpp b/dasp_amd/csrc/planio.cpp
--- a/dasp_amd/csrc/planio.cpp
+++ b/dasp_amd/csrc/planio.cpp
@@ -76,8 +76,11 @@
         for (int v : p.dst_map) if ((unsigned)v >= (unsigned)m) return fail("dst_map entry out of range");
     }
     if (p.stats.rowA != p.m || p.stats.colA != p.n || p.stats.nnzA != p.nnz || p.stats.precision != p.precision) return fail("stats header");
-    if (p.stats.row_long < 0 || p.n_mfma_rows < 0 || p.n_mfma_rows > p.stats.row_block || (long long)p.stats.row_long + p.stats.row_block > m) return fail("category counters");
-    if (n_panels == 0 && (p.med_slot0 < p.stats.row_long || (long long)p.med_slot0 + p.n_mfma_rows > (long long)p.stats.row_long + p.stats.row_block)) return fail("med_slot0");
+    const bool long_blocks = n_panels == 0 && !p.two_phase && p.stats.row_long > 0 && p.med_slot0 == 0;
+    if (p.stats.row_long < 0 || p.n_mfma_rows < 0 || (long long)p.n_mfma_rows > (long long)p.stats.row_block + (long_blocks ? p.stats.row_long : 0) ||
+        (long long)p.stats.row_long + p.stats.row_block > m) return fail("category counters");
+    if (long_blocks && (is_panel || p.windowed || p.precision != 64 || p.n_mfma_rows < p.stats.row_long || !p.piece_dst.empty() || !p.multi_dst.empty() || p.cnt_long != 0)) return fail("med_slot0: long rows as blocks");
+    if (n_panels == 0 && ((!long_blocks && p.med_slot0 < p.stats.row_long) || (long long)p.med_slot0 + p.n_mfma_rows > (long long)p.stats.row_long + p.stats.row_block)) return fail("med_slot0");
     if (p.panel_bounds.size() != 2 * (size_t)n_panels) return fail("panel_bounds size");
     if (p.two_phase) {
         if (n_panels > 0 || is_panel) return fail("two-phase plan with column panels");
@@ -139,11 +142,11 @@
         return fail("medium column ids");
     auto npair_of = [&](long long b) {
         const long long r0 = b * kMedRows, K = CH / kMedRows;
-        return med_npair((int)(p.med_ptr[(size_t)b + 1] - p.med_ptr[(size_t)b]), (int)((p.irr_ptr[(size_t)r0 + 1] - p.irr_ptr[(size_t)r0] + K - 1) / K), (int)vb, p.pair_mode);
+        return med_npair((int)(p.med_ptr[(size_t)b + 1] - p.med_ptr[(size_t)b]), (int)((med_block_tail(p.irr_ptr.data(), r0, p.n_mfma_rows) + K - 1) / K), (int)vb, p.pair_mode);
     };
     auto oneshot_of = [&](long long b) {
         const long long r0 = b * kMedRows, K = CH / kMedRows;
-        return vb == 8 && med_oneshot64((int)(p.med_ptr[(size_t)b + 1] - p.med_ptr[(size_t)b]), (int)((p.irr_ptr[(size_t)r0 + 1] - p.irr_ptr[(size_t)r0] + K - 1) / K));
+        return vb == 8 && med_oneshot64((int)(p.med_ptr[(size_t)b + 1] - p.med_ptr[(size_t)b]), (int)((med_block_tail(p.irr_ptr.data(), r0, p.n_mfma_rows) + K - 1) / K));
     };
     if (p.irr_ptr.size() != (size_t)p.n_mfma_rows + 1 || !mono(p.irr_ptr) || (size_t)p.irr_ptr.back() != p.cnt_irr) return fail("irr_ptr");
     if (p.irr_val.size() != p.cnt_irr * (size_t)vb || p.irr_cid.size() != p.cnt_irr) return fail("irregular arrays");
@@ -152,7 +155,7 @@
         if (!mono(p.med_c8ptr) || (size_t)p.med_c8ptr.back() * (size_t)CH != p.cnt_reg8) return fail("med_c8ptr");
         for (long long b = 0; b < nb; ++b) {
             const int nc = p.med_ptr[(size_t)b + 1] - p.med_ptr[(size_t)b], n8 = p.med_c8ptr[(size_t)b + 1] - p.med_c8ptr[(size_t)b], npair = npair_of(b);
-            const bool one = med_oneshot64(nc, (p.irr_ptr[(size_t)b * kMedRows + 1] - p.irr_ptr[(size_t)b * kMedRows] + 3) / 4);
+            const bool one = med_oneshot64(nc, (med_block_tail(p.irr_ptr.data(), b * kMedRows, p.n_mfma_rows) + 3) / 4);
             if (n8 < 0 || n8 > npair || n8 % (one ? 2 : kMedBatch64) || (n8 && vb != 8))
                 return fail("med_c8ptr: one-byte ids come in whole batches (pipelined) / pairs (one-shot) of an f64 block's paired region");
             std::vector<char> seen((size_t)nc, 0);
@@ -314,7 +317,7 @@
                 (p.cid16 ? p.med_val.size() == (p.med_cid16.size() + p.med_cid8.size()) * vb : p.med_val.size() == p.med_cid.size() * vb);
     if (np == 0 && !p.two_phase)
         sane = sane && p.piece_ptr.size() == p.piece_dst.size() + 1 && p.irr_ptr.size() == (size_t)p.n_mfma_rows + 1 &&
-               p.n_mfma_rows >= 0 && p.n_mfma_rows <= p.stats.row_block && (!p.windowed || p.med_dst.size() == (size_t)p.n_mfma_rows);
+               p.n_mfma_rows >= 0 && (long long)p.n_mfma_rows <= (long long)p.stats.row_block + (p.med_slot0 == 0 ? std::max(p.stats.row_long, 0) : 0) && (!p.windowed || p.med_dst.size() == (size_t)p.n_mfma_rows);
     if (!sane) return false;
     p.cnt_long = p.long_cid.size(); p.cnt_irr = p.irr_cid.size(); p.cnt_short = p.short_cid.size();
     p.cnt_long_chunks = p.long_base.size();
diff --git a/dasp_amd/csrc/sharedids.cpp b/dasp_amd/csrc/sharedids.cpp
--- a/dasp_amd/csrc/sharedids.cpp
+++ b/dasp_amd/csrc/sharedids.cpp
@@ -25,7 +25,7 @@
     for (size_t b = 0; b < nb; ++b) {
         const int c0 = p.med_ptr[b], nc = p.med_ptr[b + 1] - c0;
         const size_t r0 = b * (size_t)kMedRows;
-        const int nt = r0 + 1 < p.irr_ptr.size() ? (p.irr_ptr[r0 + 1] - p.irr_ptr[r0] + K - 1) / K : 0;
+        const int nt = r0 + 1 < p.irr_ptr.size() ? (med_block_tail(p.irr_ptr.data(), (long long)r0, (long long)p.irr_ptr.size() - 1) + K - 1) / K : 0;
         if (med_oneshot64(nc, nt)) continue;
         const int npair = med_npair(nc, nt, 8, p.pair_mode);
         if (npair <= 0) continue;
diff --git a/dasp_amd/csrc/upload.cpp b/dasp_amd/csrc/upload.cpp
--- a/dasp_amd/csrc/upload.cpp
+++ b/dasp_amd/csrc/upload.cpp
@@ -130,7 +130,7 @@
         const int K = p.geo.med_k, nbk = (int)p.med_ptr.size() - 1;
         for (int b = 0; b < nbk; ++b) {
             const int nc = p.med_ptr[(size_t)b + 1] - p.med_ptr[(size_t)b], r0 = b * kMedRows;
-            const int nt = (p.irr_ptr[(size_t)r0 + 1] - p.irr_ptr[(size_t)r0] + K - 1) / K;
+            const int nt = (med_block_tail(p.irr_ptr.data(), r0, (long long)p.irr_ptr.size() - 1) + K - 1) / K;
             all += nc + nt;
             if (med_oneshot64(nc, nt)) one += nc + nt;
         }
@@ -299,7 +299,7 @@
         const int TK = p.precision == 64 ? 4 : 16;
         for (size_t b = 0; b < med_nt.size(); ++b) {
             const size_t r0 = b * (size_t)kMedRows;
-            if (r0 + 1 < p.irr_ptr.size()) med_nt[b] = (p.irr_ptr[r0 + 1] - p.irr_ptr[r0] + TK - 1) / TK;
+            if (r0 + 1 < p.irr_ptr.size()) med_nt[b] = (med_block_tail(p.irr_ptr.data(), (long long)r0, (long long)p.irr_ptr.size() - 1) + TK - 1) / TK;
         }
     }
     const size_t o_mnt = add(med_nt.data(), med_nt.size() * 4);
diff --git a/include/dasp_amd.h b/include/dasp_amd.h
--- a/include/dasp_amd.h
+++ b/include/dasp_amd.h
@@ -70,6 +70,7 @@
     int long_cb;
     int value_map;
     int tp_exact;
+    int long_blocks;
 } dasp_options_t;
 
 void dasp_options_default(dasp_options_t *opt);
@@ -141,6 +142,7 @@
 
 int dasp_plan_shared_ids(const dasp_plan_t *plan, long long *paired_id_bytes, long long *shared_bytes, int *in_use);
 long long dasp_plan_shared_ids_export(const dasp_plan_t *plan, const char *what, void *dst, size_t bytes);
+int dasp_plan_long_blocks(const dasp_plan_t *plan, int *rows, long long *nnz);
 
 int dasp_plan_set_stream_policy(dasp_plan_t *plan, int policy);
 
```

Result: faster. 1358 GFLOP/s, median of 6 (+5.9%).
